# ZGC-SP/mpcith_kyber_kosk

Measured on AMD Instinct MI355X. Metric: kyber768_kosk_proofs_per_sec_prove_plus_verify, higher is better.
Workload: dtype u16

## Files before the change

### include/kosk_mi355x.h

```cpp
#ifndef KOSK_MI355X_H
#define KOSK_MI355X_H

#include <stddef.h>
#include <stdint.h>

#ifdef __cplusplus
extern "C" {
#endif

typedef struct kosk_ctx kosk_ctx;

typedef void (*kosk_randombytes_fn)(void *user, uint8_t *out, size_t len);

size_t kosk_pk_bytes(int kyber_k);
size_t kosk_sk_bytes(int kyber_k);
size_t kosk_proof_bytes(int kyber_k);
size_t kosk_tape_bytes(int kyber_k);
int kosk_proof_field(int kyber_k, int idx, size_t *offset, size_t *size);

#define KOSK_SEED_BYTES 32
int kosk_tape_from_seed(int kyber_k, const uint8_t seed[KOSK_SEED_BYTES], uint8_t *tape);

int kosk_create(kosk_ctx **ctx, int device, int kyber_k, int max_batch);

// ... 51 lines not shown
                        const uint8_t *tapes, size_t tape_stride, uint8_t *pi);
int kosk_verify_inst(kosk_ctx *ctx, int n, const uint8_t *pi, const uint8_t *inst, uint8_t *ok);

int kosk_stage_prover_inputs(kosk_ctx *ctx, int n, const uint8_t *tapes, size_t tape_stride, uint8_t *pk, uint8_t *sk);
int kosk_prove_resident(kosk_ctx *ctx, int n);
int kosk_fetch_proofs(kosk_ctx *ctx, int n, uint8_t *pi);
int kosk_stage_verifier_inputs(kosk_ctx *ctx, int n, const uint8_t *pi, const uint8_t *pk);
int kosk_verify_resident(kosk_ctx *ctx, int n, uint8_t *ok);
int kosk_verifiable_keygen_resident(kosk_ctx *ctx, int n, const uint8_t *tapes, size_t tape_stride, uint8_t *pk, uint8_t *sk);
int kosk_verify_resident_pk(kosk_ctx *ctx, int n, const uint8_t *pk, uint8_t *ok);
size_t kosk_compact_proof_bytes(int kyber_k);
int kosk_proof_compress(int kyber_k, const uint8_t *pi, uint8_t *out);
int kosk_proof_decompress(int kyber_k, const uint8_t *in, uint8_t *pi);
int kosk_verifiable_keygen_batch_compact(kosk_ctx *ctx, int n, const uint8_t *tapes, size_t tape_stride,
                                         uint8_t *pk, uint8_t *sk, uint8_t *out);
int kosk_verify_batch_compact(kosk_ctx *ctx, int n, const uint8_t *in, const uint8_t *pk, uint8_t *ok);
int kosk_fetch_proofs_compact(kosk_ctx *ctx, int n, uint8_t *out);
int kosk_stage_verifier_inputs_compact(kosk_ctx *ctx, int n, const uint8_t *in, const uint8_t *pk);

size_t kosk_dense_proof_bytes(int kyber_k);
int kosk_proof_dense_pack(int kyber_k, const uint8_t *pi, uint8_t *out);
int kosk_proof_dense_unpack(int kyber_k, const uint8_t *in, uint8_t *pi);
int kosk_verifiable_keygen_batch_dense(kosk_ctx *ctx, int n, const uint8_t *tapes, size_t tape_stride, uint8_t *pk, uint8_t *sk, uint8_t *out);
int kosk_verifiable_keygen_seeded_batch_dense(kosk_ctx *ctx, int n, const uint8_t *seeds, size_t seed_stride, uint8_t *pk, uint8_t *sk,
                                              uint8_t *out);
int kosk_verify_batch_dense(kosk_ctx *ctx, int n, const uint8_t *in, const uint8_t *pk, uint8_t *ok);
int kosk_fetch_proofs_dense(kosk_ctx *ctx, int n, uint8_t *out);
int kosk_stage_verifier_inputs_dense(kosk_ctx *ctx, int n, const uint8_t *in, const uint8_t *pk);
int kosk_dense_fill_device(kosk_ctx *ctx, int n, uint8_t *d_images, size_t image_stride, uint32_t *d_status);

#define KOSK_SS_BYTES 32
size_t kosk_ct_bytes(int kyber_k);
int kosk_kem_enc_batch(kosk_ctx *ctx, int n, const uint8_t *pk, const uint8_t *coins, uint8_t *ct, uint8_t *ss);
int kosk_kem_dec_batch(kosk_ctx *ctx, int n, const uint8_t *ct, const uint8_t *sk, uint8_t *ss);
int kosk_kem_enc_verified(kosk_ctx *ctx, int n, const uint8_t *coins, uint8_t *ct, uint8_t *ss, uint8_t *done);

enum { KOSK_KEM_KEY_NONE = 0, KOSK_KEM_KEY_PK = 1, KOSK_KEM_KEY_SK = 2 };
int kosk_kem_key_set(kosk_ctx *ctx, const uint8_t *pk, const uint8_t *sk);
int kosk_kem_key_state(const kosk_ctx *ctx);
int kosk_kem_key_clear(kosk_ctx *ctx);
int kosk_kem_enc_key(kosk_ctx *ctx, int n, const uint8_t *coins, uint8_t *ct, uint8_t *ss);
int kosk_kem_dec_key(kosk_ctx *ctx, int n, const uint8_t *ct, uint8_t *ss);

int kosk_kem_keypair_batch(kosk_ctx *ctx, int n, const uint8_t *coins, uint8_t *pk, uint8_t *sk);
#define KOSK_KEYCHK_HASH     1
#define KOSK_KEYCHK_PK_RANGE 2
#define KOSK_KEYCHK_S_RANGE  4
int kosk_kem_check_pk(kosk_ctx *ctx, int n, const uint8_t *pk, uint8_t *flags);
int kosk_kem_check_sk(kosk_ctx *ctx, int n, const uint8_t *sk, uint8_t *flags);

int kosk_witness_from_sk(kosk_ctx *ctx, int n, const uint8_t *sk, int16_t *se_out, uint8_t *ok);
int kosk_stage_prover_keys(kosk_ctx *ctx, int n, const uint8_t *sk, const uint8_t *tapes, size_t tape_stride, uint8_t *ok);
int kosk_stage_prover_keys_seeded(kosk_ctx *ctx, int n, const uint8_t *sk, const uint8_t *seeds, size_t seed_stride, uint8_t *ok);
int kosk_prove_keys_batch(kosk_ctx *ctx, int n, const uint8_t *sk, const uint8_t *tapes, size_t tape_stride, uint8_t *pi, uint8_t *ok);
int kosk_prove_keys_seeded_batch(kosk_ctx *ctx, int n, const uint8_t *sk, const uint8_t *seeds, size_t seed_stride, uint8_t *pi, uint8_t *ok);

int kosk_path_count(const kosk_ctx *ctx, int id, long *count);
int kosk_host_threads(const kosk_ctx *ctx);

int kosk_phase_seconds(const kosk_ctx *ctx, double *out, int n);

int kosk_profile_enable(kosk_ctx *ctx, int on);
int kosk_profile_read(const kosk_ctx *ctx, int id, double *total_ms, long *launches);
int kosk_profile_read_units(const kosk_ctx *ctx, int id, double *total_ms, long *launches, long *proofs);

int kosk_combine_stats(const kosk_ctx *ctx, long *calls, long *members);

int kosk_stream_timer_start(kosk_ctx *ctx);
int kosk_stream_timer_stop(kosk_ctx *ctx, double *ms);


int kosk_sha3_256_batch(kosk_ctx *ctx, const uint8_t *d_in, size_t in_stride, size_t inlen, uint8_t *d_out, int n);
int kosk_sha3_256_batch_pair(kosk_ctx *ctx, const uint8_t *d_in, size_t in_stride, size_t inlen, uint8_t *d_out, int n);
int kosk_sha3_256_batch_wave(kosk_ctx *ctx, const uint8_t *d_in, size_t in_stride, size_t inlen, uint8_t *d_out, int n);
int kosk_fs_alpha_device(kosk_ctx *ctx, const uint8_t *d_tables, size_t table_stride, int n, uint16_t *d_alpha, uint8_t *d_h1);
int kosk_fs_opened_device(kosk_ctx *ctx, const uint8_t *d_tables, size_t table_stride, int n, uint16_t *d_sel, uint16_t *d_rest, int sel_stride, uint8_t *d_ch);
int kosk_shake256_batch(kosk_ctx *ctx, const uint8_t *d_in, size_t in_stride, size_t inlen,
                        uint8_t *d_out, size_t outlen, int n);
int kosk_tape_expand_device(kosk_ctx *ctx, int n, const uint8_t *seeds, size_t seed_stride, uint8_t *d_tapes, size_t tape_stride);
int kosk_commit_hash_lanes(kosk_ctx *ctx, const uint16_t *d_rows, size_t row_stride, int n_lanes,
                           const uint8_t *d_prefix, int with_prefix, uint8_t *d_out);
int kosk_ntt256_batch(kosk_ctx *ctx, const int16_t *d_in, int16_t *d_out, int n);
int kosk_lagrange_expand(kosk_ctx *ctx, const uint16_t *d_y407, uint16_t *d_shares, int n);
int kosk_recon_secrets(kosk_ctx *ctx, const uint16_t *d_shares, uint16_t *d_secrets, int n, int two_d);
int kosk_device_synchronize(kosk_ctx *ctx);
int kosk_streams(const kosk_ctx *ctx);
int kosk_resident_proofs(kosk_ctx *ctx, void **d_proofs, size_t *stride);
int kosk_resident_digests(kosk_ctx *ctx, int round, void **d_digests, size_t *stride);
typedef void (*kosk_round_fn)(void *user, int role, int round, const void *d_digests, size_t bytes);
int kosk_set_round_hook(kosk_ctx *ctx, kosk_round_fn fn, void *user);


int kosk_keygen(int kyber_k, const uint8_t seed64[64], uint8_t *pk, uint8_t *sk,
                int16_t *A, int16_t *s, int16_t *e, int16_t *t);
int kosk_fs_alpha(int kyber_k, const uint8_t *tcomm_all, uint16_t *alpha);
int kosk_fs_opened(const uint8_t *digests_all, uint16_t *I, uint16_t *rest);
void kosk_host_sha3_256(uint8_t out[32], const uint8_t *in, size_t inlen);
void kosk_host_shake256(uint8_t *out, size_t outlen, const uint8_t *in, size_t inlen);
int kosk_host_sha3_256_multi(uint8_t *out, const uint8_t *in, size_t in_stride, size_t inlen, int count, int nthreads);
int kosk_lagrange_table(int which, uint16_t *out);

int kosk_bind_value(int kyber_k, const uint8_t *pk, const uint8_t context[32], uint8_t out[32]);
int kosk_bind_device(kosk_ctx *ctx, int n, const uint8_t *pk, const uint8_t *contexts, size_t context_stride, uint8_t *d_out);
int kosk_fs_alpha_bound(int kyber_k, const uint8_t *tcomm_all, const uint8_t bind[32], uint16_t *alpha);
int kosk_fs_opened_bound(const uint8_t *digests_all, const uint8_t bind[32], uint16_t *I, uint16_t *rest);
int kosk_fs_alpha_bound_device(kosk_ctx *ctx, const uint8_t *d_tables, size_t table_stride, int n, const uint8_t *d_bind, uint16_t *d_alpha, uint8_t *d_h1);
int kosk_fs_opened_bound_device(kosk_ctx *ctx, const uint8_t *d_tables, size_t table_stride, int n, const uint8_t *d_bind,
                                uint16_t *d_sel, uint16_t *d_rest, int sel_stride, uint8_t *d_ch);
int kosk_set_contexts(kosk_ctx *ctx, int n, const uint8_t *contexts, size_t context_stride);

int kosk_keyseed_value(int kyber_k, const uint8_t *sk, const uint8_t *context, const uint8_t *salt, uint8_t seed[32]);
int kosk_keyseed_device(kosk_ctx *ctx, int n, const uint8_t *sk, const uint8_t *contexts, size_t context_stride,
                        const uint8_t *salts, size_t salt_stride, uint8_t *d_seeds);
int kosk_stage_prover_keys_derived(kosk_ctx *ctx, int n, const uint8_t *sk, const uint8_t *salts, size_t salt_stride, uint8_t *ok);
int kosk_prove_keys_derived_batch(kosk_ctx *ctx, int n, const uint8_t *sk, const uint8_t *salts, size_t salt_stride, uint8_t *pi, uint8_t *ok);

#ifdef __cplusplus
}
#endif
#endif
```

### mpcith_kyber_kosk_amd/api.py

```python
import ctypes as C
import os

from . import build as _build

_HERE = os.path.dirname(os.path.abspath(__file__))
LIB_PATH = os.environ.get("KOSK_LIB_PATH") or os.path.join(_HERE, "libkosk_mi355x.so")


class KoskError(RuntimeError):
    pass


def _load():
    if not os.path.exists(LIB_PATH):
        _build.build()
    lib = C.CDLL(LIB_PATH)
    u8p, u16p, i16p, sz, vp = C.POINTER(C.c_uint8), C.POINTER(C.c_uint16), C.POINTER(C.c_int16), C.c_size_t, C.c_void_p
    sig = {
        "kosk_pk_bytes": (sz, [C.c_int]), "kosk_sk_bytes": (sz, [C.c_int]),
        "kosk_proof_bytes": (sz, [C.c_int]), "kosk_tape_bytes": (sz, [C.c_int]),
        "kosk_proof_field": (C.c_int, [C.c_int, C.c_int, C.POINTER(sz), C.POINTER(sz)]),
        "kosk_create": (C.c_int, [C.POINTER(vp), C.c_int, C.c_int, C.c_int]),
        "kosk_options_init": (None, [vp]),
        "kosk_create_ex": (C.c_int, [C.POINTER(vp), C.c_int, C.c_int, C.c_int, vp]),
# ... 63 lines not shown
        "kosk_set_entropy": (C.c_int, [vp, C.c_int]),
        "kosk_tape_expand_device": (C.c_int, [vp, C.c_int, vp, sz, vp, sz]),
        "kosk_verifiable_keygen_seeded_batch": (C.c_int, [vp, C.c_int, vp, sz, vp, vp, vp]),
        "kosk_verifiable_keygen_seeded_batch_compact": (C.c_int, [vp, C.c_int, vp, sz, vp, vp, vp]),
        "kosk_verifiable_keygen_seeded_resident": (C.c_int, [vp, C.c_int, vp, sz, vp, vp]),
        "kosk_stage_prover_inputs_seeded": (C.c_int, [vp, C.c_int, vp, sz, vp, vp]),
    }
    if not (os.environ.get("KOSK_LIB_PATH") and not hasattr(lib, "kosk_tape_from_seed")):
        sig.update(seeded)
    kem = {
        "kosk_ct_bytes": (sz, [C.c_int]),
        "kosk_kem_enc_batch": (C.c_int, [vp, C.c_int, vp, vp, vp, vp]),
        "kosk_kem_dec_batch": (C.c_int, [vp, C.c_int, vp, vp, vp]),
        "kosk_kem_enc_verified": (C.c_int, [vp, C.c_int, vp, vp, vp, vp]),
    }
    if not (os.environ.get("KOSK_LIB_PATH") and not hasattr(lib, "kosk_kem_enc_batch")):
        sig.update(kem)
    keyproof = {
        "kosk_witness_from_sk": (C.c_int, [vp, C.c_int, vp, vp, vp]),
        "kosk_stage_prover_keys": (C.c_int, [vp, C.c_int, vp, vp, sz, vp]),
        "kosk_stage_prover_keys_seeded": (C.c_int, [vp, C.c_int, vp, vp, sz, vp]),
        "kosk_prove_keys_batch": (C.c_int, [vp, C.c_int, vp, vp, sz, vp, vp]),
        "kosk_prove_keys_seeded_batch": (C.c_int, [vp, C.c_int, vp, vp, sz, vp, vp]),
    }
    if not (os.environ.get("KOSK_LIB_PATH") and not hasattr(lib, "kosk_witness_from_sk")):
        sig.update(keyproof)
    bound = {
        "kosk_bind_value": (C.c_int, [C.c_int, vp, vp, vp]),
        "kosk_bind_device": (C.c_int, [vp, C.c_int, vp, vp, sz, vp]),
        "kosk_fs_alpha_bound": (C.c_int, [C.c_int, vp, vp, vp]),
        "kosk_fs_opened_bound": (C.c_int, [vp, vp, vp, vp]),
        "kosk_fs_alpha_bound_device": (C.c_int, [vp, vp, sz, C.c_int, vp, vp, vp]),
        "kosk_fs_opened_bound_device": (C.c_int, [vp, vp, sz, C.c_int, vp, vp, vp, C.c_int, vp]),
        "kosk_set_contexts": (C.c_int, [vp, C.c_int, vp, sz]),
    }
    if not (os.environ.get("KOSK_LIB_PATH") and not hasattr(lib, "kosk_set_contexts")):
        sig.update(bound)
    dense = {
        "kosk_dense_proof_bytes": (sz, [C.c_int]),
        "kosk_proof_dense_pack": (C.c_int, [C.c_int, vp, vp]),
        "kosk_proof_dense_unpack": (C.c_int, [C.c_int, vp, vp]),
        "kosk_fetch_proofs_dense": (C.c_int, [vp, C.c_int, vp]),
        "kosk_stage_verifier_inputs_dense": (C.c_int, [vp, C.c_int, vp, vp]),
        "kosk_verifiable_keygen_batch_dense": (C.c_int, [vp, C.c_int, vp, sz, vp, vp, vp]),
        "kosk_verifiable_keygen_seeded_batch_dense": (C.c_int, [vp, C.c_int, vp, sz, vp, vp, vp]),
        "kosk_verify_batch_dense": (C.c_int, [vp, C.c_int, vp, vp, vp]),
        "kosk_dense_fill_device": (C.c_int, [vp, C.c_int, vp, sz, vp]),
    }
    if not (os.environ.get("KOSK_LIB_PATH") and not hasattr(lib, "kosk_dense_proof_bytes")):
        sig.update(dense)
    keypair = {
        "kosk_kem_keypair_batch": (C.c_int, [vp, C.c_int, vp, vp, vp]),
        "kosk_kem_check_pk": (C.c_int, [vp, C.c_int, vp, vp]),
        "kosk_kem_check_sk": (C.c_int, [vp, C.c_int, vp, vp]),
    }
    if not (os.environ.get("KOSK_LIB_PATH") and not hasattr(lib, "kosk_kem_keypair_batch")):
        sig.update(keypair)
    keyseed = {
        "kosk_keyseed_value": (C.c_int, [C.c_int, vp, vp, vp, vp]),
        "kosk_keyseed_device": (C.c_int, [vp, C.c_int, vp, vp, sz, vp, sz, vp]),
        "kosk_stage_prover_keys_derived": (C.c_int, [vp, C.c_int, vp, vp, sz, vp]),
        "kosk_prove_keys_derived_batch": (C.c_int, [vp, C.c_int, vp, vp, sz, vp, vp]),
    }
    if not (os.environ.get("KOSK_LIB_PATH") and not hasattr(lib, "kosk_keyseed_value")):
        sig.update(keyseed)
    wipe = {
        "kosk_wipe_secrets": (C.c_int, [vp]),
        "kosk_set_wipe": (C.c_int, [vp, C.c_int]),
        "kosk_secret_scan": (C.c_int, [vp, vp, sz, C.POINTER(C.c_long)]),
        "kosk_wipe_device": (C.c_int, [vp, C.c_int, vp, vp]),
        "kosk_wipe_timing": (C.c_int, [vp, C.c_int, C.POINTER(C.c_double), C.POINTER(C.c_double), C.POINTER(C.c_size_t), C.POINTER(C.c_int)]),
    }
    if not (os.environ.get("KOSK_LIB_PATH") and not hasattr(lib, "kosk_wipe_secrets")):
        sig.update(wipe)
    onekey = {
        "kosk_kem_key_set": (C.c_int, [vp, vp, vp]),
        "kosk_kem_key_state": (C.c_int, [vp]),
        "kosk_kem_key_clear": (C.c_int, [vp]),
        "kosk_kem_enc_key": (C.c_int, [vp, C.c_int, vp, vp, vp]),
        "kosk_kem_dec_key": (C.c_int, [vp, C.c_int, vp, vp]),
    }
    if not (os.environ.get("KOSK_LIB_PATH") and not hasattr(lib, "kosk_kem_key_set")):
        sig.update(onekey)
    for name, (res, args) in sig.items():
        fn = getattr(lib, name)
        fn.restype = res
        fn.argtypes = args
    return lib


lib = _load()
EXPORTS = ["kosk_pk_bytes", "kosk_sk_bytes", "kosk_proof_bytes", "kosk_tape_bytes", "kosk_proof_field", "kosk_create",
           "kosk_destroy", "kosk_last_error", "kosk_set_randombytes", "kosk_verifiable_keygen_batch", "kosk_verify_batch",
           "kosk_verify_fail_masks", "kosk_randomness_bytes", "kosk_range_proof_bytes", "kosk_mlwe_inst_bytes",
           "kosk_prepare_randomness", "kosk_prepare_range_proof", "kosk_prove_prepared", "kosk_verify_inst", "kosk_compact_proof_bytes",
           "kosk_proof_compress", "kosk_proof_decompress", "kosk_fetch_proofs_compact", "kosk_stage_verifier_inputs_compact", "kosk_stage_prover_inputs", "kosk_prove_resident", "kosk_fetch_proofs",
           "kosk_stage_verifier_inputs", "kosk_verify_resident", "kosk_verifiable_keygen_resident", "kosk_verify_resident_pk",
           "kosk_resident_digests", "kosk_set_round_hook", "kosk_phase_seconds", "kosk_path_count", "kosk_host_threads", "kosk_sha3_256_batch_pair", "kosk_verifiable_keygen_batch_compact", "kosk_verify_batch_compact", "kosk_host_alloc", "kosk_host_free", "kosk_sha3_256_batch",
           "kosk_shake256_batch", "kosk_commit_hash_lanes", "kosk_ntt256_batch", "kosk_lagrange_expand",
           "kosk_recon_secrets", "kosk_profile_enable", "kosk_profile_read", "kosk_profile_read_units", "kosk_combine_stats", "kosk_stream_timer_start", "kosk_stream_timer_stop", "kosk_device_synchronize", "kosk_streams", "kosk_resident_proofs", "kosk_keygen", "kosk_fs_alpha",
           "kosk_fs_opened", "kosk_host_sha3_256", "kosk_host_shake256", "kosk_host_sha3_256_multi", "kosk_lagrange_table",
           "kosk_options_init", "kosk_create_ex", "kosk_sha3_256_batch_wave", "kosk_fs_alpha_device", "kosk_fs_opened_device",
           "kosk_tape_from_seed", "kosk_set_entropy", "kosk_tape_expand_device", "kosk_verifiable_keygen_seeded_batch",
           "kosk_verifiable_keygen_seeded_batch_compact", "kosk_verifiable_keygen_seeded_resident", "kosk_stage_prover_inputs_seeded",
           "kosk_ct_bytes", "kosk_kem_enc_batch", "kosk_kem_dec_batch", "kosk_kem_enc_verified",
           "kosk_witness_from_sk", "kosk_stage_prover_keys", "kosk_stage_prover_keys_seeded", "kosk_prove_keys_batch",
           "kosk_prove_keys_seeded_batch",
           "kosk_bind_value", "kosk_bind_device", "kosk_fs_alpha_bound", "kosk_fs_opened_bound", "kosk_fs_alpha_bound_device",
           "kosk_fs_opened_bound_device", "kosk_set_contexts",
           "kosk_dense_proof_bytes", "kosk_proof_dense_pack", "kosk_proof_dense_unpack", "kosk_fetch_proofs_dense",
           "kosk_stage_verifier_inputs_dense", "kosk_verifiable_keygen_batch_dense", "kosk_verifiable_keygen_seeded_batch_dense",
           "kosk_verify_batch_dense", "kosk_dense_fill_device",
           "kosk_kem_keypair_batch", "kosk_kem_check_pk", "kosk_kem_check_sk",
           "kosk_keyseed_value", "kosk_keyseed_device", "kosk_stage_prover_keys_derived", "kosk_prove_keys_derived_batch",
           "kosk_wipe_secrets", "kosk_set_wipe", "kosk_secret_scan", "kosk_wipe_device", "kosk_wipe_timing",
           "kosk_kem_key_set", "kosk_kem_key_state", "kosk_kem_key_clear", "kosk_kem_enc_key", "kosk_kem_dec_key"]
HAS_KEM = hasattr(lib, "kosk_kem_enc_batch")


class KoskOptions(C.Structure):
    _fields_ = [("size", C.c_uint32), ("streams", C.c_int32), ("combine", C.c_int32), ("combine_wait_us", C.c_int32),
                ("combine_idle_us", C.c_int32), ("combine_prewake_us", C.c_int32), ("strict_encoding", C.c_int32), ("fs_mode", C.c_int32),
                ("host_threads", C.c_int32), ("blocking_sync", C.c_int32), ("hooks_unmerged", C.c_int32), ("reserved", C.c_int32 * 6)]


FS_HOST, FS_DEVICE = 0, 1
ENTROPY_TAPE, ENTROPY_SEED = 0, 1
WIPE_OFF, WIPE_CALL = 0, 1
SEED_BYTES = 32
SS_BYTES = 32
KEYPAIR_COIN_BYTES = 64
KEYCHK_HASH, KEYCHK_PK_RANGE, KEYCHK_S_RANGE = 1, 2, 4
KEM_KEY_NONE, KEM_KEY_PK, KEM_KEY_SK = 0, 1, 2


def options(**fields):
    o = KoskOptions()
    lib.kosk_options_init(C.byref(o))
    for k_, v_ in fields.items():
        if k_ not in dict(KoskOptions._fields_) or k_ in ("size", "reserved"):
            raise KoskError("unknown option " + k_)
        setattr(o, k_, int(v_))
    return o


def pk_bytes(k): return lib.kosk_pk_bytes(k)
def sk_bytes(k): return lib.kosk_sk_bytes(k)
def proof_bytes(k): return lib.kosk_proof_bytes(k)
def tape_bytes(k): return lib.kosk_tape_bytes(k)
def ct_bytes(k): return lib.kosk_ct_bytes(k)
def dense_proof_bytes(k): return lib.kosk_dense_proof_bytes(k)


def dense_pack(k, pi):
    if len(pi) != proof_bytes(k):
        raise KoskError("dense_pack: an image of kosk_proof_bytes")
    out = C.create_string_buffer(dense_proof_bytes(k))
    rc = lib.kosk_proof_dense_pack(k, C.c_char_p(bytes(pi)), out)
    return rc, out.raw


def dense_unpack(k, rec):
    if len(rec) != dense_proof_bytes(k):
        raise KoskError("dense_unpack: a record of kosk_dense_proof_bytes")
    out = C.create_string_buffer(proof_bytes(k))
    rc = lib.kosk_proof_dense_unpack(k, C.c_char_p(bytes(rec)), out)
    return rc, out.raw


CONTEXT_BYTES = 32


def bind_value(k, pk, context):
    pk, context = bytes(pk), bytes(context)
    if len(pk) != pk_bytes(k) or len(context) != CONTEXT_BYTES:
        raise KoskError("bind_value: a public key of kosk_pk_bytes and a context of %d bytes" % CONTEXT_BYTES)
    out = C.create_string_buffer(32)
    if lib.kosk_bind_value(k, C.c_char_p(pk), C.c_char_p(context), out):
        raise KoskError("kosk_bind_value: kyber_k outside 2..4")
    return out.raw


SALT_BYTES = 32


def keyseed_value(k, sk, context=None, salt=None):
    sk = bytes(sk)
    if len(sk) != sk_bytes(k):
        raise KoskError("keyseed_value: a secret key of kosk_sk_bytes")
    if context is not None and len(context) != CONTEXT_BYTES:
        raise KoskError("a context has %d bytes" % CONTEXT_BYTES)
    if salt is not None and len(salt) != SALT_BYTES:
        raise KoskError("a salt has %d bytes" % SALT_BYTES)
    out = C.create_string_buffer(SEED_BYTES)
    cp = None if context is None else C.c_char_p(bytes(context))
    sp = None if salt is None else C.c_char_p(bytes(salt))
    if lib.kosk_keyseed_value(k, C.c_char_p(sk), cp, sp, out):
        raise KoskError("kosk_keyseed_value: kyber_k outside 2..4")
    return out.raw
# ... 331 lines not shown
    def verify_inst(self, proofs, insts):
        n = len(proofs)
        ok = (C.c_uint8 * n)()
        self._chk(lib.kosk_verify_inst(self._h, n, b"".join(proofs), b"".join(insts), ok), "verify_inst")
        return [bool(x) for x in ok]

    def stage_prover_inputs(self, tapes=None, n=None, seeds=None, seed_stride=None):
        if seeds is not None:
            sp, ss, n, _keep = self._seed_arg(seeds, n, seed_stride)
            self._pk = C.create_string_buffer(self.pk_bytes * n); self._sk = C.create_string_buffer(self.sk_bytes * n)
            self._chk(lib.kosk_stage_prover_inputs_seeded(self._h, n, sp, ss, self._pk, self._sk), "stage_prover_inputs")
            return n
        if tapes is not None:
            n = len(tapes)
        blob = b"".join(t[:self.tape_bytes] for t in tapes) if tapes is not None else None
        self._pk = C.create_string_buffer(self.pk_bytes * n); self._sk = C.create_string_buffer(self.sk_bytes * n)
        self._chk(lib.kosk_stage_prover_inputs(self._h, n, C.c_char_p(blob) if blob is not None else None, self.tape_bytes, self._pk, self._sk), "stage_prover_inputs")
        return n

    def prove_resident(self, n):
        self._chk(lib.kosk_prove_resident(self._h, n), "prove_resident")

    def verify_resident(self, n):
        ok = C.create_string_buffer(n)
        self._chk(lib.kosk_verify_resident(self._h, n, ok), "verify_resident")
        return [b == 1 for b in ok.raw]

    def fetch_proofs(self, n):
        pi = C.create_string_buffer(self.proof_bytes * n)
        self._chk(lib.kosk_fetch_proofs(self._h, n, pi), "fetch_proofs")
        return [pi.raw[i * self.proof_bytes:(i + 1) * self.proof_bytes] for i in range(n)]

    def verifiable_keygen_resident(self, tapes=None, n=None, tape_stride=None, seeds=None, seed_stride=None):
        if seeds is not None:
            sp, ss, n, _keep = self._seed_arg(seeds, n, seed_stride)
            if getattr(self, "_pk", None) is None or len(self._pk) != self.pk_bytes * n:
                self._pk = C.create_string_buffer(self.pk_bytes * n); self._sk = C.create_string_buffer(self.sk_bytes * n)
            self._chk(lib.kosk_verifiable_keygen_seeded_resident(self._h, n, sp, ss, self._pk, self._sk), "verifiable_keygen_resident")
            return n
        if isinstance(tapes, int):
            tp, stride = C.c_void_p(tapes), tape_stride
        elif tapes is None:
            tp, stride = None, 0
        else:
            n = len(tapes)
            blob = b"".join(t[:self.tape_bytes] for t in tapes)
            tp, stride = C.c_char_p(blob), self.tape_bytes
        if getattr(self, "_pk", None) is None or len(self._pk) != self.pk_bytes * n:
            self._pk = C.create_string_buffer(self.pk_bytes * n); self._sk = C.create_string_buffer(self.sk_bytes * n)
        self._chk(lib.kosk_verifiable_keygen_resident(self._h, n, tp, stride, self._pk, self._sk), "verifiable_keygen_resident")
        return n

    def keys(self, n):
        return ([self._pk.raw[i * self.pk_bytes:(i + 1) * self.pk_bytes] for i in range(n)],
                [self._sk.raw[i * self.sk_bytes:(i + 1) * self.sk_bytes] for i in range(n)])

    def verify_resident_pk(self, n, pks=None):
        ok = C.create_string_buffer(n)
        self._chk(lib.kosk_verify_resident_pk(self._h, n, C.c_char_p(b"".join(pks)) if pks is not None else None, ok), "verify_resident_pk")
        return [b == 1 for b in ok.raw]

    def resident_digests(self, rnd, n):
        d, stride = C.c_void_p(), C.c_size_t()
        self._chk(lib.kosk_resident_digests(self._h, rnd, C.byref(d), C.byref(stride)), "resident_digests")
        assert stride.value == 1454 * 32
        return DeviceView(d.value, (n, 1454, 32))

    def set_round_hook(self, fn):
        if fn is None:
            self._hook = None
            self._chk(lib.kosk_set_round_hook(self._h, None, None), "set_round_hook")
            return
        CB = C.CFUNCTYPE(None, C.c_void_p, C.c_int, C.c_int, C.c_void_p, C.c_size_t)
        self._hook = CB(lambda _u, role, rnd, ptr, nbytes: fn(role, rnd, ptr, nbytes))
        self._chk(lib.kosk_set_round_hook(self._h, C.cast(self._hook, C.c_void_p), None), "set_round_hook")

    def phase_seconds(self):
        out = (C.c_double * 16)()
        lib.kosk_phase_seconds(self._h, out, 16)
        return list(out)

    PROFILE_IDS = ["hash_tcomm", "hash_view", "gemm_expand1", "gemm_expand2", "lincomb", "ntt_f", "assemble",
                   "v_hash_tcomm", "v_hash_view", "v_interp_build", "v_gemm_interp", "v_gemm_expand", "v_gemm_recon", "v_lincomb",
                   "fs_alpha", "fs_opened", "v_fs_alpha", "v_fs_opened"]

    def profile_enable(self, on=True):
        self._chk(lib.kosk_profile_enable(self._h, int(on)), "profile_enable")

    def profile_read(self):
        out = {}
        for i, name in enumerate(self.PROFILE_IDS):
            ms, cnt = C.c_double(), C.c_long()
            lib.kosk_profile_read(self._h, i, C.byref(ms), C.byref(cnt))
            out[name] = (ms.value, cnt.value)
        return out

    def profile_read_units(self):
        out = {}
        for i, name in enumerate(self.PROFILE_IDS):
            ms, cnt, units = C.c_double(), C.c_long(), C.c_long()
            lib.kosk_profile_read_units(self._h, i, C.byref(ms), C.byref(cnt), C.byref(units))
            out[name] = (ms.value, cnt.value, units.value)
        return out

    def combine_stats(self):
        a, b = C.c_long(), C.c_long()
        self._chk(lib.kosk_combine_stats(self._h, C.byref(a), C.byref(b)), "combine_stats")
        return a.value, b.value

    def _records(self, what, x, n, size):
        if isinstance(x, int):
            if n is None:
                raise KoskError("a device pointer for %s needs n" % what)
            return C.c_void_p(x), n, None
        for r_ in x:
            if len(r_) != size:
                raise KoskError("a %s record has %d bytes" % (what, size))
        blob = b"".join(bytes(r_) for r_ in x)
        return C.c_char_p(blob), len(x), blob

    def _kem_out(self, out, n, sizes):
        if out is not None:
            if len(out) != len(sizes):
                raise KoskError("out needs %d device pointers" % len(sizes))
            return [C.c_void_p(int(p_)) for p_ in out], None
        bufs = [C.create_string_buffer(s_ * n) for s_ in sizes]
        return bufs, bufs

    def kem_enc(self, pks, coins=None, n=None, out=None):
        pp, n, _k1 = self._records("pk", pks, n, self.pk_bytes)
        cp, _k2 = None, None
        if coins is not None:
            cp, nc, _k2 = self._records("coins", coins, n, 32)
            if nc != n:
                raise KoskError("coins for %d items, public keys for %d" % (nc, n))
        ctb = ct_bytes(self.k)
        bufs, host = self._kem_out(out, n, (ctb, SS_BYTES))
        self._chk(lib.kosk_kem_enc_batch(self._h, n, pp, cp, bufs[0], bufs[1]), "kem_enc")
        if host is None:
            return out
        return _cut(bufs[0], ctb, n), _cut(bufs[1], SS_BYTES, n)

    def kem_dec(self, cts, sks, n=None, out=None):
        ctb = ct_bytes(self.k)
        cp, n, _k1 = self._records("ct", cts, n, ctb)
        sp, ns, _k2 = self._records("sk", sks, n, self.sk_bytes)
        if ns != n:
            raise KoskError("secret keys for %d items, ciphertexts for %d" % (ns, n))
        bufs, host = self._kem_out(None if out is None else (out,), n, (SS_BYTES,))
        self._chk(lib.kosk_kem_dec_batch(self._h, n, cp, sp, bufs[0]), "kem_dec")
        if host is None:
            return out
        return _cut(bufs[0], SS_BYTES, n)

    def kem_keypair(self, coins=None, n=None, out=None):
        cp, _k = None, None
        if coins is not None:
            cp, n, _k = self._records("coins", coins, n, KEYPAIR_COIN_BYTES)
        elif n is None:
            n = 1
        bufs, host = self._kem_out(out, n, (self.pk_bytes, self.sk_bytes))
        self._chk(lib.kosk_kem_keypair_batch(self._h, n, cp, bufs[0], bufs[1]), "kem_keypair")
        if host is None:
            return out
        return _cut(bufs[0], self.pk_bytes, n), _cut(bufs[1], self.sk_bytes, n)

    def _kem_check(self, fn, what, recs, n, size):
# ... 43 lines not shown
        self._chk(lib.kosk_kem_enc_key(self._h, n, cp, bufs[0], bufs[1]), "kem_enc_key")
        if host is None:
            return out
        return _cut(bufs[0], ctb, n), _cut(bufs[1], SS_BYTES, n)

    def kem_dec_key(self, cts, n=None, out=None):
        ctb = ct_bytes(self.k)
        cp, n, _k = self._records("ct", cts, n, ctb)
        bufs, host = self._kem_out(None if out is None else (out,), n, (SS_BYTES,))
        self._chk(lib.kosk_kem_dec_key(self._h, n, cp, bufs[0]), "kem_dec_key")
        if host is None:
            return out
        return _cut(bufs[0], SS_BYTES, n)

    def witness_from_sk(self, sks, n=None):
        import numpy as np
        sp, n, _keep = self._records("sk", sks, n, self.sk_bytes)
        se = np.zeros((n, 2 * self.k, 256), np.int16)
        ok = C.create_string_buffer(n)
        self._chk(lib.kosk_witness_from_sk(self._h, n, sp, se.ctypes.data, ok), "witness_from_sk")
        return se, [b == 1 for b in ok.raw[:n]]

    def _key_rand(self, tapes, seeds, n, seed_stride):
        if seeds is not None:
            sp, ss, ns, keep = self._seed_arg(seeds, n, seed_stride)
            if ns != n:
                raise KoskError("seeds for %d proofs, secret keys for %d" % (ns, n))
            return True, sp, ss, keep
        if tapes is None:
            return False, None, 0, None
        if isinstance(tapes, int):
            return False, C.c_void_p(tapes), self.tape_bytes, None
        if len(tapes) != n:
            raise KoskError("tapes for %d proofs, secret keys for %d" % (len(tapes), n))
        for t in tapes:
            if len(t) < self.tape_bytes:
                raise KoskError("tape shorter than kosk_tape_bytes")
        blob = b"".join(t[:self.tape_bytes] for t in tapes)
        return False, C.c_char_p(blob), self.tape_bytes, blob

    def stage_prover_keys(self, sks, tapes=None, seeds=None, n=None, seed_stride=None, derived=False, salts=None, salt_stride=None):
        sp, n, _k1 = self._records("sk", sks, n, self.sk_bytes)
        if derived or salts is not None:
            if tapes is not None or seeds is not None:
                raise KoskError("derived=True takes neither tapes nor seeds")
            rp, stride, _k2 = self._salt_arg(salts, n, salt_stride)
            ok = C.create_string_buffer(n)
            self._chk(lib.kosk_stage_prover_keys_derived(self._h, n, sp, rp, stride, ok), "stage_prover_keys")
            return [b == 1 for b in ok.raw[:n]]
        seeded, rp, stride, _k2 = self._key_rand(tapes, seeds, n, seed_stride)
        ok = C.create_string_buffer(n)
        fn = lib.kosk_stage_prover_keys_seeded if seeded else lib.kosk_stage_prover_keys
        self._chk(fn(self._h, n, sp, rp, stride, ok), "stage_prover_keys")
        return [b == 1 for b in ok.raw[:n]]

    def prove_keys(self, sks, tapes=None, seeds=None, n=None, seed_stride=None, derived=False, salts=None, salt_stride=None):
        sp, n, _k1 = self._records("sk", sks, n, self.sk_bytes)
        if derived or salts is not None:
            if tapes is not None or seeds is not None:
                raise KoskError("derived=True takes neither tapes nor seeds")
            rp, stride, _k2 = self._salt_arg(salts, n, salt_stride)
            ok = C.create_string_buffer(n)
            pi = C.create_string_buffer(self.proof_bytes * n)
            self._chk(lib.kosk_prove_keys_derived_batch(self._h, n, sp, rp, stride, pi, ok), "prove_keys")
            return _cut(pi, self.proof_bytes, n), [b == 1 for b in ok.raw[:n]]
        seeded, rp, stride, _k2 = self._key_rand(tapes, seeds, n, seed_stride)
        ok = C.create_string_buffer(n)
        pi = C.create_string_buffer(self.proof_bytes * n)
        fn = lib.kosk_prove_keys_seeded_batch if seeded else lib.kosk_prove_keys_batch
        self._chk(fn(self._h, n, sp, rp, stride, pi, ok), "prove_keys")
        return _cut(pi, self.proof_bytes, n), [b == 1 for b in ok.raw[:n]]

    PATH_IDS = ["hash_dma", "hash_plain", "table_gemm", "limb_gemm", "copy_direct", "copy_staged", "graph_replay", "digest_copy", "small_copy_kernel",
                "fs_device", "fs_host", "tape_expand", "kem_enc", "kem_dec"]

    PATH_DENSE_FILL = 14
    PATH_KEM_KEYPAIR = 15
    PATH_KEM_CHECK = 16
    PATH_KEYSEED = 17
    PATH_WIPE = 18
    PATH_KEM_KEY_SETUP = 19
    PATH_KEM_ENC_KEY = 20
    PATH_KEM_DEC_KEY = 21

    def path_count(self, path_id):
        v = C.c_long()
        self._chk(lib.kosk_path_count(self._h, int(path_id), C.byref(v)), "path_count")
        return v.value

    def path_counts(self):
        out = {}
        for i, name in enumerate(self.PATH_IDS if HAS_KEM else self.PATH_IDS[:12]):
            v = C.c_long()
            self._chk(lib.kosk_path_count(self._h, i, C.byref(v)), "path_count")
            out[name] = v.value
        return out

    @property
    def host_threads(self):
        return lib.kosk_host_threads(self._h)

    def timer_start(self):
        self._chk(lib.kosk_stream_timer_start(self._h), "timer_start")

    def timer_stop_ms(self):
        ms = C.c_double()
        self._chk(lib.kosk_stream_timer_stop(self._h, C.byref(ms)), "timer_stop")
        return ms.value

    @property
    def streams(self):
        return lib.kosk_streams(self._h)

    def synchronize(self):
        self._chk(lib.kosk_device_synchronize(self._h), "synchronize")

    def sha3_256_batch(self, d_in, in_stride, inlen, d_out, n):
        self._chk(lib.kosk_sha3_256_batch(self._h, d_in, in_stride, inlen, d_out, n), "sha3_256_batch")

    def sha3_256_batch_pair(self, d_in, in_stride, inlen, d_out, n):
        self._chk(lib.kosk_sha3_256_batch_pair(self._h, d_in, in_stride, inlen, d_out, n), "sha3_256_batch_pair")

    def sha3_256_batch_wave(self, d_in, in_stride, inlen, d_out, n):
        self._chk(lib.kosk_sha3_256_batch_wave(self._h, d_in, in_stride, inlen, d_out, n), "sha3_256_batch_wave")

    def fs_alpha_device(self, d_tables, table_stride, n, d_alpha, d_h1=None):
        self._chk(lib.kosk_fs_alpha_device(self._h, d_tables, table_stride, n, d_alpha, d_h1), "fs_alpha_device")

    def fs_opened_device(self, d_tables, table_stride, n, d_sel, d_rest, sel_stride, d_ch=None):
        self._chk(lib.kosk_fs_opened_device(self._h, d_tables, table_stride, n, d_sel, d_rest, sel_stride, d_ch), "fs_opened_device")

    def fs_alpha_bound_device(self, d_tables, table_stride, n, d_bind, d_alpha, d_h1=None):
        self._chk(lib.kosk_fs_alpha_bound_device(self._h, d_tables, table_stride, n, d_bind, d_alpha, d_h1), "fs_alpha_bound_device")

    def fs_opened_bound_device(self, d_tables, table_stride, n, d_bind, d_sel, d_rest, sel_stride, d_ch=None):
        self._chk(lib.kosk_fs_opened_bound_device(self._h, d_tables, table_stride, n, d_bind, d_sel, d_rest, sel_stride, d_ch), "fs_opened_bound_device")

    def shake256_batch(self, d_in, in_stride, inlen, d_out, outlen, n):
        self._chk(lib.kosk_shake256_batch(self._h, d_in, in_stride, inlen, d_out, outlen, n), "shake256_batch")

    def commit_hash_lanes(self, d_rows, row_stride, n_lanes, d_prefix, with_prefix, d_out):
        self._chk(lib.kosk_commit_hash_lanes(self._h, d_rows, row_stride, n_lanes, d_prefix, int(with_prefix), d_out), "commit_hash_lanes")

    def ntt256_batch(self, d_in, d_out, n):
        self._chk(lib.kosk_ntt256_batch(self._h, d_in, d_out, n), "ntt256_batch")

    def lagrange_expand(self, d_y407, d_shares, n):
        self._chk(lib.kosk_lagrange_expand(self._h, d_y407, d_shares, n), "lagrange_expand")

    def recon_secrets(self, d_shares, d_secrets, n, two_d=False):
        self._chk(lib.kosk_recon_secrets(self._h, d_shares, d_secrets, n, int(two_d)), "recon_secrets")
```

### mpcith_kyber_kosk_amd/csrc/kosk_capi.cpp

```cpp
#include "../../include/kosk_mi355x.h"

#include <unistd.h>

#include <algorithm>
#include <condition_variable>
#include <cstdio>
#include <cstring>
#include <exception>
#include <functional>
#include <memory>
#include <mutex>
#include <string>
#include <thread>
#include <vector>

#include "kosk_combine.hpp"
#include "kosk_ctx.hpp"
#include "kosk_lanes.hpp"

using namespace kosk;

struct kosk_ctx;
struct Cohort {
    int device = 0, k = 0, per = 0;
// ... 1723 lines not shown
    return 0;
    GUARD_END
}
int kosk_fs_opened_bound_device(kosk_ctx *ctx, const uint8_t *d_tables, size_t table_stride, int n, const uint8_t *d_bind, uint16_t *d_sel, uint16_t *d_rest,
                                int sel_stride, uint8_t *d_ch)
{
    if (!ctx || !d_tables || !d_sel || !d_rest || !d_bind || n < 1 || sel_stride < NREST || sel_stride < SEL_OPOS + NOPEN ||
        (reinterpret_cast<uintptr_t>(d_tables) & 7) || (table_stride & 7) || (reinterpret_cast<uintptr_t>(d_bind) & 7)) return bad_args(ctx, __func__);
    GUARD(ctx)
    Ctx &c = *ctx->c;
    ctx->clear_err();
    HIPCHK_C(hipSetDevice(c.device));
    FsArgs fa{};
    fa.in = d_tables; fa.in_stride = table_stride; fa.len = NPARTY * 32; fa.out_digest = d_ch;
    fa.I = d_sel; fa.rest = d_rest; fa.sel_stride = sel_stride; fa.bind = d_bind;
    HIPCHK_C(launch_fs_chain(fa, FS_OPENED, n, c.stream));
    return 0;
    GUARD_END
}

int kosk_commit_hash_lanes(kosk_ctx *ctx, const uint16_t *d_rows, size_t row_stride, int n_lanes,
                           const uint8_t *d_prefix, int with_prefix, uint8_t *d_out)
{
    if (!ctx) return -1;
    GUARD(ctx)
    Ctx &c = *ctx->c;
    ctx->clear_err();
    HIPCHK_C(hipSetDevice(c.device));
    HashArgs ha{};
    ha.rows = d_rows;
    ha.group_stride = 0;
    ha.row_stride = (int)row_stride;
    ha.col_off = 0;
    ha.lanes_per_group = n_lanes;
    ha.prefix = d_prefix;
    ha.out = d_out;
    ha.out_lanes_per_group = n_lanes;
    int variant = 0;
    HIPCHK_C(launch_commit_hash(ha, 1, c.P.K, with_prefix != 0, c.stream, &variant));
    c.path_n[(variant & 1) ? PATH_HASH_DMA : PATH_HASH_PLAIN]++;
    return 0;
    GUARD_END
}

int kosk_ntt256_batch(kosk_ctx *ctx, const int16_t *d_in, int16_t *d_out, int n)
{
    if (!ctx) return -1;
    GUARD(ctx)
    Ctx &c = *ctx->c;
    ctx->clear_err();
    HIPCHK_C(hipSetDevice(c.device));
    NttArgs na{};
    na.in = d_in;
    na.out = d_out;
    na.npg = n;
    na.npoly = n;
    na.out_canonical = 0;
    HIPCHK_C(launch_ntt(na, c.stream));
    return 0;
    GUARD_END
}

int kosk_lagrange_expand(kosk_ctx *ctx, const uint16_t *d_y407, uint16_t *d_shares, int n)
{
    if (!ctx) return -1;
    GUARD(ctx)
    Ctx &c = *ctx->c;
    ctx->clear_err();
    HIPCHK_C(hipSetDevice(c.device));
    const int cap = c.own_batch * c.rm.nrows;
    for (int done = 0; done < n;) {
        const int m = (n - done) < cap ? (n - done) : cap;
        HIPCHK_C(launch_rows_copy(d_y407 + (size_t)done * XLEN, XLEN, c.d_P, RS, XLEN, m, c.stream));
        const GemmSrc gs{c.d_P, 0, nullptr, RS, 0, 0};
        const GemmDst gd{c.d_P, 0, nullptr, RS, EXP_OFF};
        if (gemm_modq(c, c.t_expand, gs, gd, m, 1)) return -1;
        HIPCHK_C(launch_rows_copy(c.d_P + NSEC, RS, d_shares + (size_t)done * NPARTY, NPARTY, NPARTY, m, c.stream));
        done += m;
    }
    return 0;
    GUARD_END
}

int kosk_recon_secrets(kosk_ctx *ctx, const uint16_t *d_shares, uint16_t *d_secrets, int n, int two_d)
{
    if (!ctx) return -1;
    GUARD(ctx)
    Ctx &c = *ctx->c;
    ctx->clear_err();
    HIPCHK_C(hipSetDevice(c.device));
    const GemmTable &t = two_d ? c.t_recon_2d : c.t_recon_d;
    const int cap = c.own_batch * c.rm.nrows;
    for (int done = 0; done < n;) {
        const int m = (n - done) < cap ? (n - done) : cap;
        HIPCHK_C(launch_rows_copy(d_shares + (size_t)done * NPARTY, NPARTY, c.d_P + NSEC, RS, NPARTY, m, c.stream));
        const GemmSrc gs{c.d_P, 0, nullptr, RS, NSEC, 0};
        const GemmDst gd{c.d_P, 0, nullptr, RS, 0};
        if (gemm_modq(c, t, gs, gd, m, 1)) return -1;
        HIPCHK_C(launch_rows_copy(c.d_P, RS, d_secrets + (size_t)done * NSEC, NSEC, NSEC, m, c.stream));
        done += m;
    }
    return 0;
    GUARD_END
}


int kosk_keygen(int kyber_k, const uint8_t seed64[64], uint8_t *pk, uint8_t *sk, int16_t *A, int16_t *s, int16_t *e, int16_t *t)
{
    Params P;
    if (!make_params(kyber_k, P) || !seed64 || !pk || !sk) return -1;
    return guard(static_cast<const kosk_ctx *>(nullptr), __func__, [&]() -> int {
    std::unique_ptr<HostKey> key(new HostKey());
    struct Gone { HostKey *k; ~Gone() { host_wipe(k, sizeof(HostKey)); } } gone{key.get()};
    host_keygen(P, seed64, pk, sk, *key);
    const int K = P.K;
    if (A) memcpy(A, key->A, sizeof(int16_t) * K * K * 256);
    if (s) memcpy(s, key->se, sizeof(int16_t) * K * 256);
    if (e) memcpy(e, key->se + K * 256, sizeof(int16_t) * K * 256);
    if (t) memcpy(t, key->t, sizeof(int16_t) * K * 256);
    return 0;
    GUARD_END
}

int kosk_fs_alpha(int kyber_k, const uint8_t *tcomm_all, uint16_t *alpha)
{
    Params P;
    if (!make_params(kyber_k, P) || !tcomm_all || !alpha) return -1;
    return guard(static_cast<const kosk_ctx *>(nullptr), __func__, [&]() -> int {
    fs_alpha(P, tcomm_all, alpha);
    return 0;
    GUARD_END
}

int kosk_fs_opened(const uint8_t *digests_all, uint16_t *I, uint16_t *rest)
{
    if (!digests_all || !I || !rest) return -1;
    return guard(static_cast<const kosk_ctx *>(nullptr), __func__, [&]() -> int {
    fs_opened(digests_all, I, rest);
    return 0;
    GUARD_END
}

int kosk_bind_value(int kyber_k, const uint8_t *pk, const uint8_t context[32], uint8_t out[32])
{
    Params P;
    if (!make_params(kyber_k, P) || !pk || !context || !out) return -1;
    return guard(static_cast<const kosk_ctx *>(nullptr), __func__, [&]() -> int {
    bind_value(P, pk, context, out);
    return 0;
    GUARD_END
}
int kosk_keyseed_value(int kyber_k, const uint8_t *sk, const uint8_t *context, const uint8_t *salt, uint8_t seed[32])
{
    Params P;
    if (!make_params(kyber_k, P) || !sk || !seed) return -1;
    return guard(static_cast<const kosk_ctx *>(nullptr), __func__, [&]() -> int {
    keyseed_value(P, sk, context, salt, seed);
    return 0;
    GUARD_END
}
int kosk_fs_alpha_bound(int kyber_k, const uint8_t *tcomm_all, const uint8_t bind[32], uint16_t *alpha)
{
    Params P;
    if (!make_params(kyber_k, P) || !tcomm_all || !bind || !alpha) return -1;
    return guard(static_cast<const kosk_ctx *>(nullptr), __func__, [&]() -> int {
    fs_alpha(P, tcomm_all, alpha, bind);
// ... 51 lines not shown
```

### mpcith_kyber_kosk_amd/csrc/kosk_ctx.cpp

```cpp
#include "kosk_ctx.hpp"

#include <atomic>

#include <chrono>
#include <cstdio>
#include <cstring>
#include <ctime>
#include <thread>

#include "kosk_math.hpp"

namespace kosk {

#define HIPCHK(x) KOSK_HIPCHK(x)

static double now_sec()
{
    return std::chrono::duration<double>(std::chrono::steady_clock::now().time_since_epoch()).count();
}

template <typename T>
static hipError_t dalloc(T **p, size_t n)
{
    return hipMalloc(reinterpret_cast<void **>(p), n * sizeof(T));
}
template <typename T>
static hipError_t halloc(T **p, size_t n)
{
    return hipHostMalloc(reinterpret_cast<void **>(p), n * sizeof(T), hipHostMallocDefault);
}

void Ctx::prof_collect()
{
    if (!prof_on) return;
    for (int i = 0; i < PR_COUNT; i++)
        if (prof_used[i]) {
            float ms = 0;
            if (hipEventElapsedTime(&ms, prof_ev[i][0], prof_ev[i][1]) == hipSuccess) { prof_ms[i] += ms; prof_n[i]++; prof_units[i] += prof_cur_units[i]; }
            prof_used[i] = false;
        }
}

Ctx::~Ctx()
{
    for (auto &g : seg)
        if (g.exec) (void)hipGraphExecDestroy(g.exec);
    for (auto &pe : prof_ev)
        for (auto e : pe)
            if (e) (void)hipEventDestroy(e);
    if (ev_sync) (void)hipEventDestroy(ev_sync);
    kem_release(*this);
    kem_key_release(*this);
    witness_release(*this);
    if (is_view) {
        if (h_err) (void)hipHostFree(h_err);
        if (d_compact) (void)hipFree(d_compact);
        if (d_compact_bad) (void)hipFree(d_compact_bad);
        if (h_compact) (void)hipHostFree(h_compact);
        if (h_compact_bad) (void)hipHostFree(h_compact_bad);
        if (d_dense_ws) (void)hipFree(d_dense_ws);
        if (d_dense_status) (void)hipFree(d_dense_status);
        if (pool) pool_destroy(pool);
        if (ev) (void)hipEventDestroy(ev);
        if (ev_kg) (void)hipEventDestroy(ev_kg);
        for (auto e : timer_ev)
            if (e) (void)hipEventDestroy(e);
        return;
    }
    void *dev[] = {t_expand.dfrag, t_recon_d.dfrag, t_recon_2d.dfrag, d_fresh_rows, d_gemm1_rows, d_gemm2_rows, d_off, d_fields, d_asm_groups, d_asm_elems,
                   d_rowtab, d_P, d_tape, d_seedbuf, d_dig1, d_dig2, d_proof, d_A, d_se, d_kg, d_sehat, d_t, d_alpha, d_I, d_pwT, d_coef, d_lin_rows,
                   d_gather, d_gather2, d_O, d_w, d_ell, d_sec, d_sec_u1, d_sec_u2, d_fail, d_inv, d_invlimb, d_vfields,
                   d_vrowtab, d_rows_bg, d_rows_isrc, d_rows_idst, d_rows_u, d_fact, d_invfact, d_node_of, d_isort, d_hrange, d_odig, d_bind};
    for (void *p : dev)
        if (p) (void)hipFree(p);
    void *host[] = {h_err, h_tape, h_seedbuf, h_dig, h_dig2, h_proof, h_alpha, h_I, h_fail, h_Iimg, h_kg, h_odig, h_bind};
    for (void *p : host)
        if (p) (void)hipHostFree(p);
    if (d_compact) (void)hipFree(d_compact);
    if (d_compact_bad) (void)hipFree(d_compact_bad);
    if (h_compact) (void)hipHostFree(h_compact);
    if (h_compact_bad) (void)hipHostFree(h_compact_bad);
    if (d_dense_ws) (void)hipFree(d_dense_ws);
    if (d_dense_status) (void)hipFree(d_dense_status);
    if (pool) pool_destroy(pool);
    if (ev) (void)hipEventDestroy(ev);
    if (ev_kg) (void)hipEventDestroy(ev_kg);
    for (auto e : timer_ev)
        if (e) (void)hipEventDestroy(e);
    if (stream) (void)hipStreamDestroy(stream);
}

static void pack_frag_table(const std::vector<uint16_t> &A, int M, int Kdim, int Mpad, int KS, std::vector<uint8_t> &out)
{
    const int RT = Mpad / 16;
    out.assign((size_t)KS * RT * 2048, 0);
    for (int m = 0; m < M; m++)
        for (int k = 0; k < Kdim; k++) {
            int c0, c1;
            limb_split(gf_center(A[(size_t)m * Kdim + k]), c0, c1);
            out[frag_offset(m, k, 0, RT)] = (uint8_t)(int8_t)c0;
            out[frag_offset(m, k, 1, RT)] = (uint8_t)(int8_t)c1;
        }
}

static int upload_table(Ctx &c, GemmTable &t, const std::vector<uint16_t> &A, int M, int Kdim)
{
    t.M = M;
    t.Mpad = (M + 127) / 128 * 128;
    t.KS = (Kdim + 63) / 64;
    std::vector<uint8_t> pk;
    pack_frag_table(A, M, Kdim, t.Mpad, t.KS, pk);
    HIPCHK(dalloc(&t.dfrag, pk.size()));
    c.reg_buf("table", &t.dfrag, pk.size(), 0);
    HIPCHK(hipMemcpyAsync(t.dfrag, pk.data(), pk.size(), hipMemcpyHostToDevice, c.stream));
    HIPCHK(hipStreamSynchronize(c.stream));
    return 0;
}

static hipError_t commit_hash_batch(Ctx &c, const HashArgs &ha, int n, int K, bool view, hipStream_t st)
{
    c.prof_begin(view ? PR_HASH_VIEW : PR_HASH_TCOMM, n);
    int variant = 0;
    const hipError_t e = launch_commit_hash(ha, n, K, view, st, &variant);
    if (!c.capturing) c.path_n[(variant & 1) ? PATH_HASH_DMA : PATH_HASH_PLAIN]++;
    c.prof_end(view ? PR_HASH_VIEW : PR_HASH_TCOMM);
    return e;
}

int device_error_check(Ctx &c)
{
    if (!c.h_err) return 0;
    const uint32_t e = *reinterpret_cast<volatile uint32_t *>(c.h_err);
    if (!e) return 0;
    *reinterpret_cast<volatile uint32_t *>(c.h_err) = 0;
    c.err = (e & DEVERR_XOF_BLOCKS) ? "gen_matrix: SHAKE128 block limit reached before 256 coefficients were accepted (indcpa.c:124-145 would squeeze on; "
                                      "probability < 2^-300 with the default limit of 32 blocks): no result was produced"
                                    : "a kernel reported an internal error";
    return -1;
}

int bind_check(Ctx &c, int n)
{
    if (c.bind_n > 0 && (c.bind_first < 0 || c.bind_first + n > c.bind_n)) {
        c.err = "the handle is armed with fewer contexts than this call has proofs (kosk_set_contexts)";
        return -1;
    }
    return 0;
}

int issue_bind_values(Ctx &c, int n)
{
    if (c.bind_n <= 0) return 0;
    if (bind_check(c, n)) return -1;
    BindArgs ba{};
    ba.pk = c.d_pk; ba.pk_stride = c.pk_stride; ba.pk_bytes = (int)c.P.pk_bytes; ba.K = c.P.K;
    ba.contexts = c.bind_ctx + (size_t)c.bind_first * 32;
    ba.out = c.d_bind;
    HIPCHK(launch_bind_values(ba, n, c.stream));
    if (!c.fs_device) HIPCHK(copy_small(c, c.h_bind, 0, c.d_bind, 0, (size_t)n * 32, 1, hipMemcpyDeviceToHost, c.stream));
    return 0;
}

hipError_t copy_round_table(Ctx &c, uint8_t *h_dst, const uint8_t *d_src, int n)
{
    return hipMemcpyAsync(h_dst, d_src, (size_t)n * NPARTY * 32, hipMemcpyDeviceToHost, c.stream);
}

hipError_t copy_small(Ctx &c, void *dst, size_t dst_stride, const void *src, size_t src_stride, size_t row_bytes, size_t nrows, hipMemcpyKind kind, hipStream_t st)
{
    if (!row_bytes || !nrows) return hipSuccess;
    if (copy_small_ok(src, src_stride, dst, dst_stride, row_bytes)) {
        if (!c.capturing) c.path_n[PATH_SMALL_COPY_KERNEL]++;
        return launch_copy_small(src, src_stride, dst, dst_stride, row_bytes, nrows, st);
    }
    if (nrows == 1 || (src_stride == row_bytes && dst_stride == row_bytes)) return hipMemcpyAsync(dst, src, row_bytes * nrows, kind, st);
    return hipMemcpy2DAsync(dst, dst_stride, src, src_stride, row_bytes, nrows, kind, st);
}

hipError_t stream_sync(Ctx &c)
{
    if (!c.blocking_sync) return hipStreamSynchronize(c.stream);
    const hipError_t e = hipEventRecord(c.ev_sync, c.stream);
    return e != hipSuccess ? e : hipEventSynchronize(c.ev_sync);
}

hipError_t wait_event(Ctx &c, hipEvent_t ev, int site, int n)
{
// ... 6 lines not shown
    if (!h) {
        h = lru;
        *h = Ctx::WaitHist{};
        h->n = n;
    }
    h->stamp = ++c.wait_stamp;
    int filled = 0;
    double est = 0;
    for (int i = 0; i < Ctx::WAIT_HIST; i++)
        if (h->us[i] > 0) { est = filled ? (h->us[i] < est ? h->us[i] : est) : h->us[i]; filled++; }
    const double t0 = now_sec();
    bool overslept = false;
    if (filled >= 4 && est > 250.0) {
        const double keep = est * 0.3 > 100.0 ? est * 0.3 : 100.0;
        double nap_us = est - keep;
        if (nap_us > 200000.0) nap_us = 200000.0;
        struct timespec ts;
        ts.tv_sec = 0;
        ts.tv_nsec = (long)(nap_us * 1e3);
        nanosleep(&ts, nullptr);
        const hipError_t q = hipEventQuery(ev);
        if (q == hipSuccess) overslept = true;
        else if (q != hipErrorNotReady) return q;
    }
    const hipError_t e = overslept ? hipSuccess : hipEventSynchronize(ev);
    const double took = (now_sec() - t0) * 1e6;
    if (overslept) {
        for (int i = 0; i < Ctx::WAIT_HIST; i++) h->us[i] = 0;
        h->at = 0;
    } else {
        h->us[h->at] = took > 1.0 ? took : 1.0;
        h->at = (h->at + 1) % Ctx::WAIT_HIST;
    }
    return e;
}
hipError_t stream_sync_site(Ctx &c, int site, int n)
{
    if (c.blocking_sync || !c.wait_nap) return stream_sync(c);
    const hipError_t e = hipEventRecord(c.ev_sync, c.stream);
    return e != hipSuccess ? e : wait_event(c, c.ev_sync, site, n);
}

int gemm_modq(Ctx &c, const GemmTable &t, const GemmSrc &s, const GemmDst &d, int npg, int ngroups)
{
    if (npg <= 0 || ngroups <= 0) return 0;
    GemmArgs ga{};
    ga.Afrag = t.dfrag; ga.Mpad = t.Mpad; ga.M = t.M; ga.KS = t.KS;
    ga.src = s.src; ga.src_gstride = s.gstride; ga.src_rows = s.rows; ga.src_rstride = s.rstride; ga.src_koff = s.koff;
    ga.src_canonical = s.canonical;
    ga.C = d.C; ga.c_gstride = d.gstride; ga.c_rows = d.rows; ga.c_rstride = d.rstride; ga.c_off = d.off;
    ga.npg = npg; ga.ngroups = ngroups;
    if (!table_gemm_ok(ga)) { c.err = "internal: table_gemm_ok() refuses the operands of a mod-q product"; return -1; }
    HIPCHK(launch_table_gemm(ga, c.stream));
    if (!c.capturing) c.path_n[PATH_TABLE_GEMM]++;
    return 0;
}

template <typename T>
static int upload_vec(Ctx &c, T **d, const std::vector<T> &v)
{
    HIPCHK(dalloc(d, v.size() ? v.size() : 1));
    c.reg_buf("table", d, v.size() * sizeof(T), 0);
    if (!v.empty()) {
        HIPCHK(hipMemcpyAsync(*d, v.data(), v.size() * sizeof(T), hipMemcpyHostToDevice, c.stream));
        HIPCHK(hipStreamSynchronize(c.stream));
    }
    return 0;
}

static int build_tables(Ctx &c)
{
    const Params &P = c.P;
    const RowMap &rm = c.rm;
    const int K = P.K, M = P.M, E = P.E, Z = P.Z;

    {
        std::vector<uint16_t> A((size_t)EXP_M * XLEN, 0);
        for (int m = 0; m < EXP_M; m++) {
            const int x = EXP_OFF + m;
            if (x < XLEN) A[(size_t)m * XLEN + x] = 1;
            else if (x < NPTS) lagrange_row(&A[(size_t)m * XLEN], XLEN, 0, x);
        }
        if (upload_table(c, c.t_expand, A, EXP_M, XLEN)) return -1;
    }
    {
        std::vector<uint16_t> A((size_t)NSEC * XLEN), A2((size_t)NSEC * (DEG2 + 1));
        for (int i = 0; i < NSEC; i++) {
            lagrange_row(&A[(size_t)i * XLEN], XLEN, NSEC, i);
            lagrange_row(&A2[(size_t)i * (DEG2 + 1)], DEG2 + 1, NSEC, i);
        }
        if (upload_table(c, c.t_recon_d, A, NSEC, XLEN)) return -1;
        if (upload_table(c, c.t_recon_2d, A2, NSEC, DEG2 + 1)) return -1;
    }

    std::vector<int16_t> fresh;
    for (int i = 0; i < M; i++) { fresh.push_back((int16_t)(rm.f + i)); fresh.push_back((int16_t)(rm.tf + i)); }
    for (int i = 0; i < K; i++)
        for (int j = 0; j < E; j++) { fresh.push_back((int16_t)(rm.seta + i * E + j)); fresh.push_back((int16_t)(rm.eeta + i * E + j)); }
    for (int i = 0; i < K; i++) { fresh.push_back((int16_t)(rm.s + i)); fresh.push_back((int16_t)(rm.e + i)); }
    for (int i = 0; i < K; i++) fresh.push_back((int16_t)(rm.nttas + i));
    for (int i = 0; i < K; i++)
        for (int j = 0; j < Z; j++) { fresh.push_back((int16_t)rm.zs(i, j)); fresh.push_back((int16_t)rm.ze(i, j)); }
    if ((int)fresh.size() != P.nfresh) { c.err = "internal: fresh row count"; return -1; }
    if (upload_vec(c, &c.d_fresh_rows, fresh)) return -1;
    if (upload_vec(c, &c.d_gemm1_rows, fresh)) return -1;
    c.n_gemm1 = (int)fresh.size();
    std::vector<int16_t> g2;
    for (int i = 0; i < K; i++) { g2.push_back((int16_t)(rm.nttsr + i)); g2.push_back((int16_t)(rm.ntter + i)); g2.push_back((int16_t)(rm.nttasr + i)); }
    if (upload_vec(c, &c.d_gemm2_rows, g2)) return -1;
    c.n_gemm2 = (int)g2.size();

    {
        std::vector<int16_t> lr(256, 0);
        for (int j = 0; j < P.J; j++) {
            lr[j] = (int16_t)(j < NCHK ? rm.beta(j) : rm.r + (j - NCHK));
            lr[128 + j] = (int16_t)(j < NCHK ? rm.gamma(j) : rm.nttr + (j - NCHK));
        }
        if (upload_vec(c, &c.d_lin_rows, lr)) return -1;
    }

    std::vector<int32_t> off;
    auto push_rows = [&](int row0, int n) { int b = (int)off.size(); for (int i = 0; i < n; i++) off.push_back((row0 + i) * RS); return b; };
    c.off_ntt1_src = push_rows(rm.f, M);
    push_rows(rm.s, K);
    c.off_ntt1_dst = push_rows(rm.tf, M);
    push_rows(rm.shat, K);
    c.n_ntt1 = M + K;
    c.off_sr_er = push_rows(rm.sr, 2 * K);
    c.off_nttsr_er = push_rows(rm.nttsr, 2 * K);
    if (rm.er != rm.sr + K || rm.ntter != rm.nttsr + K) { c.err = "internal: row map adjacency"; return -1; }
    if (upload_vec(c, &c.d_off, off)) return -1;

    auto add = [&](int fid, int sel, int width, auto rowfn) {
        FieldDesc fd{};
        fd.off = (uint32_t)P.off[fid];
        fd.sel = sel;
        fd.width = width;
        fd.rowtab_off = (int)c.h_rowtab.size();
        for (int e = 0; e < width; e++) c.h_rowtab.push_back((int16_t)rowfn(e));
        c.h_fields.push_back(fd);
    };
    add(F_F, 0, M, [&](int e) { return rm.f + e; });
    add(F_NTTF, 0, M, [&](int e) { return rm.tf + e; });
    add(F_BETA, 1, NCHK, [&](int e) { return rm.beta(e); });
    add(F_GAMMA, 1, NCHK, [&](int e) { return rm.gamma(e); });
    add(F_S, 0, K, [&](int e) { return rm.s + e; });
    add(F_E, 0, K, [&](int e) { return rm.e + e; });
    add(F_T, 1, K, [&](int e) { return rm.t + e; });
    add(F_NTTS, 0, K, [&](int e) { return rm.ntts + e; });
    add(F_NTTE, 0, K, [&](int e) { return rm.ntte + e; });
    add(F_NTTAR, 0, K, [&](int e) { return rm.nttar + e; });
    add(F_NTTAS, 0, K, [&](int e) { return rm.nttas + e; });
    add(F_SR, 1, K, [&](int e) { return rm.sr + e; });
    add(F_ER, 1, K, [&](int e) { return rm.er + e; });
    add(F_SETA, 1, K * E, [&](int e) { return rm.seta + e; });
    add(F_EETA, 1, K * E, [&](int e) { return rm.eeta + e; });
    add(F_SSUB, 0, K * E, [&](int e) { return rm.ssub + e; });
    add(F_ESUB, 0, K * E, [&](int e) { return rm.esub + e; });
    add(F_ZS, 0, K * Z, [&](int e) { return rm.zs(e / Z, e % Z); });
    add(F_ZE, 0, K * Z, [&](int e) { return rm.ze(e / Z, e % Z); });
    add(F_US, 1, K * Z, [&](int e) { return rm.us(e / Z, e % Z); });
    add(F_UE, 1, K * Z, [&](int e) { return rm.ue(e / Z, e % Z); });
    c.nfields = (int)c.h_fields.size();
    c.pplan = make_field_plan(c.h_fields.data(), c.nfields);
    {
        std::vector<AsmGroup> groups;
        std::vector<AsmElem> elems;
        for (int sel = 1; sel >= 0; sel--) {
            AsmGroup g{};
            auto flush = [&]() {
                if (g.nsub) groups.push_back(g);
                g = AsmGroup{};
            };
            for (int f = 0; f < c.nfields; f++) {
                const FieldDesc &fd = c.h_fields[f];
                if (fd.sel != sel) continue;
                if (g.nsub && (g.nrows + fd.width > 80 || g.nsub == 12)) flush();
                if (!g.nsub) { g.sel = sel; g.rowtab_off = (int)c.h_rowtab.size(); g.elem_off = (int)elems.size(); }
                g.sub_off[g.nsub] = fd.off; g.sub_width[g.nsub] = (int16_t)fd.width; g.sub_col[g.nsub] = (int16_t)g.nrows;
                for (int k = 0; k < fd.width; k++) {
                    c.h_rowtab.push_back(c.h_rowtab[fd.rowtab_off + k]);
                    elems.push_back(AsmElem{(int32_t)(fd.off / 2 + k), (int16_t)fd.width, (int16_t)(64 * g.nrows + k)});
                }
                g.nrows += fd.width;
                g.nsub++;
            }
            flush();
        }
        if ((int)groups.size() > ASM_MAX_GROUPS) { c.err = "internal: image field groups"; return -1; }
        for (int i = 0; i < 128; i++) elems.push_back(AsmElem{0, 1, 0});
        c.n_asm_groups = (int)groups.size();
        if (upload_vec(c, &c.d_asm_groups, groups)) return -1;
        if (upload_vec(c, &c.d_asm_elems, elems)) return -1;
    }
    if (upload_vec(c, &c.d_fields, c.h_fields)) return -1;
    if (upload_vec(c, &c.d_rowtab, c.h_rowtab)) return -1;
    return 0;
}

int ctx_create(Ctx **out, int device, int kyber_k, int max_batch, std::string &err, int host_share, const CtxOpts &opts)
{
    Ctx *cp = new Ctx();
    Ctx &c = *cp;
    auto fail = [&]() { err = c.err; delete cp; return -1; };
    if (!make_params(kyber_k, c.P)) { c.err = "kyber_k must be 2, 3 or 4"; return fail(); }
    if (max_batch < 1) { c.err = "max_batch must be >= 1"; return fail(); }
    int ndev = 0;
    if (hipGetDeviceCount(&ndev) != hipSuccess || ndev <= 0) {
        (void)hipGetLastError();
        c.err = "no HIP device available: the KOSK path has no CPU fallback";
        return fail();
    }
    if (device < 0 || device >= ndev) {
        c.err = "device " + std::to_string(device) + " out of range: " + std::to_string(ndev) + " HIP device(s) visible";
        return fail();
    }
    c.device = device;
    c.max_batch = max_batch;
    c.rm = make_rowmap(c.P);
    const int cpus = host_cpu_count() / (host_share > 0 ? host_share : 1);
    c.nthreads = cpus > 8 ? 8 : (cpus < 1 ? 1 : cpus);
    if (opts.host_threads > 0) c.nthreads = opts.host_threads > 64 ? 64 : opts.host_threads;
    c.pool = pool_create();
    c.nthreads = pool_reserve(c.pool, c.nthreads);
    c.base_threads = c.nthreads;
    c.reserved_threads = c.nthreads;
    c.own_batch = max_batch;
    c.call_cap = max_batch;
    if (const char *e = getenv("KOSK_GRAPHS")) c.use_graphs = atoi(e) != 0;
    if (const char *e = getenv("KOSK_WAIT_NAP")) c.wait_nap = atoi(e) != 0;
    if (const char *e = getenv("KOSK_REGISTER")) c.host_register = atoi(e) != 0;
    if (const char *e = getenv("KOSK_DEBUG_XOF_BLOCKS")) c.xof_max_blocks = atoi(e) > 0 ? atoi(e) : c.xof_max_blocks;
    if (opts.blocking_sync >= 0) c.blocking_sync = opts.blocking_sync != 0;
    if (opts.strict_encoding >= 0) c.strict_encoding = opts.strict_encoding != 0;
    if (opts.fs_device >= 0) c.fs_device = opts.fs_device != 0;

    auto body = [&]() -> int {
        HIPCHK(hipSetDevice(device));
        {
            int cus = 0;
            HIPCHK(hipDeviceGetAttribute(&cus, hipDeviceAttributeMultiprocessorCount, device));
            if (cus > 0) c.n_simd = 4 * cus;
        }
        HIPCHK(hipStreamCreateWithFlags(&c.stream, hipStreamNonBlocking));
        HIPCHK(hipEventCreateWithFlags(&c.ev, hipEventDisableTiming | (c.blocking_sync ? hipEventBlockingSync : 0)));
        HIPCHK(hipEventCreateWithFlags(&c.ev_kg, hipEventDisableTiming | (c.blocking_sync ? hipEventBlockingSync : 0)));
        if (c.blocking_sync) HIPCHK(hipEventCreateWithFlags(&c.ev_sync, hipEventDisableTiming | hipEventBlockingSync));
        else if (c.wait_nap) HIPCHK(hipEventCreateWithFlags(&c.ev_sync, hipEventDisableTiming));
        for (auto &pe : c.prof_ev)
            for (auto &e : pe) HIPCHK(hipEventCreate(&e));
        if (build_tables(c)) return -1;
        const Params &P = c.P;
        const size_t B = (size_t)max_batch;
        c.proof_stride = (size_t)c.rm.nrows * RS;
        c.tape_stride = (P.tape_bytes + 63) / 64 * 64;
        c.image_stride = (P.proof_bytes + 63) / 64 * 64;
        c.key_stride = (size_t)P.K * P.K * 256;
        c.se_stride = (size_t)2 * P.K * 256;
        c.sel_stride = 1312;
        auto dev = [&](auto **p, size_t per) -> hipError_t {
            const hipError_t e = dalloc(p, B * per);
            if (e == hipSuccess) { c.reg_pp(p, per * sizeof(**p)); c.reg_buf("workspace", p, per * sizeof(**p), Ctx::INV_PER_PROOF); }
            return e;
        };
        auto host = [&](auto **p, size_t per) -> hipError_t {
// ... 800 lines not shown
```

### mpcith_kyber_kosk_amd/csrc/kosk_ctx.hpp

```cpp
#pragma once
#include <hip/hip_runtime.h>

#include <string>
#include <functional>
#include <vector>

#include "kosk_device.hpp"
#include "kosk_host.hpp"
#include "kosk_params.hpp"

#define KOSK_HIPCHK(x)                                                      \
    do {                                                                    \
        hipError_t e_ = (x);                                                \
        if (e_ != hipSuccess) {                                             \
            (void)hipGetLastError();                                        \
            c.err = std::string(#x) + ": " + hipGetErrorString(e_);         \
            return -1;                                                      \
        }                                                                   \
    } while (0)

namespace kosk {

typedef void (*randombytes_fn)(void *user, uint8_t *out, size_t len);
typedef void (*round_fn)(void *user, int role, int round, const void *d_digests, size_t bytes);

struct KeygenIn {
    const uint8_t *tapes;
    size_t tape_stride;
    uint8_t *pk, *sk;
    int count = 0;
    const KeygenIn *next = nullptr;
    round_fn hook = nullptr;
    void *hook_user = nullptr;
    const uint8_t *seeds = nullptr;
    size_t seed_stride = 0;
};
struct VerifySeg {
    int count;
    const uint8_t *pk;
    uint8_t *ok;
    const VerifySeg *next = nullptr;
    round_fn hook = nullptr;
    void *hook_user = nullptr;
};

enum Phase { PH_HOST_PRE = 0, PH_GPU_COMMIT, PH_FS_ALPHA, PH_GPU_RELATION, PH_FS_OPEN, PH_GPU_ASSEMBLE, PH_D2H,
             PH_P1_ISSUE, PH_P2_ISSUE, PH_P3_ISSUE, PH_V1_ISSUE, PH_V1_WAIT, PH_V_FS_ALPHA, PH_V2_ISSUE, PH_V2_WAIT, PH_V_FS_OPEN,
             PH_COUNT };

enum ProfId { PR_HASH_TCOMM = 0, PR_HASH_VIEW, PR_GEMM_EXPAND1, PR_GEMM_EXPAND2, PR_LINCOMB, PR_NTT_F, PR_ASSEMBLE,
              PR_V_HASH_TCOMM, PR_V_HASH_VIEW, PR_V_INTERP_BUILD, PR_V_GEMM_INTERP, PR_V_GEMM_EXPAND, PR_V_GEMM_RECON,
              PR_V_LINCOMB, PR_FS_ALPHA, PR_FS_OPENED, PR_V_FS_ALPHA, PR_V_FS_OPENED, PR_COUNT };

enum PathId { PATH_HASH_DMA = 0, PATH_HASH_PLAIN, PATH_TABLE_GEMM, PATH_LIMB_GEMM, PATH_COPY_DIRECT, PATH_COPY_STAGED,
              PATH_GRAPH_REPLAY, PATH_DIGEST_COPY, PATH_SMALL_COPY_KERNEL, PATH_FS_DEVICE, PATH_FS_HOST, PATH_TAPE_EXPAND, PATH_KEM_ENC, PATH_KEM_DEC, PATH_DENSE_FILL, PATH_KEM_KEYPAIR, PATH_KEM_CHECK, PATH_KEYSEED, PATH_WIPE,
              PATH_KEM_KEY_SETUP, PATH_KEM_ENC_KEY, PATH_KEM_DEC_KEY, PATH_COUNT };

struct GemmTable {
    uint8_t *dfrag = nullptr;
    int M = 0, Mpad = 0, KS = 0;
};

struct GemmSrc {
    const uint16_t *src;
    size_t gstride;
    const int16_t *rows;
    int rstride, koff;
    int canonical = 1;
};
struct GemmDst {
    uint16_t *C;
    size_t gstride;
    const int16_t *rows;
    int rstride, off;
};

struct CompactField {
    uint32_t src_off, dst_off, n;
    int raw;
};
struct CompactPlan {
    CompactField f[NFIELDS];
    size_t bytes;
};
CompactPlan make_compact_plan(const Params &P);
int compact_encode(const Params &P, const uint8_t *img, uint8_t *out);
void compact_decode(const Params &P, const uint8_t *in, uint8_t *img);
CompactPlan make_dense_plan(const Params &P);
int dense_encode(const Params &P, const uint8_t *img, uint8_t *out);
int dense_decode(const Params &P, const uint8_t *in, uint8_t *img);

struct KemWs;
struct KemKey;
enum { KEM_CHUNK = 16384,
       KEM_WAVE_MAX = 1024 };

struct Ctx {
    int device = 0;
    Params P{};
    RowMap rm{};
    int max_batch = 0;
    struct PerProof { size_t field_off, stride_bytes; };
    std::vector<PerProof> per_proof;
    template <class T> void reg_pp(T **field, size_t stride_bytes)
    {
        per_proof.push_back({(size_t)(reinterpret_cast<char *>(field) - reinterpret_cast<char *>(this)), stride_bytes});
    }
    enum { INV_HOST = 1, INV_SECRET = 2, INV_PER_PROOF = 4 };
    enum { INVG_CORE = 0, INVG_VERIFY, INVG_COMPACT, INVG_DENSE, INVG_KEM, INVG_WITNESS, INVG_BIND, INVG_KEMKEY };
    struct InvBuf {
        const char *name;
        size_t field_off;
        void *abs;
        size_t bytes;
        size_t sec_off, sec_bytes;
        int flags, group;
    };
    std::vector<InvBuf> inv;
    template <class T> void reg_buf(const char *name, T **field, size_t bytes, int flags, int group = INVG_CORE, size_t sec_off = 0, size_t sec_bytes = (size_t)-1)
    {
        const char *f = reinterpret_cast<const char *>(field), *me = reinterpret_cast<const char *>(this);
        const bool mine = f >= me && f < me + sizeof(*this);
        inv.push_back(InvBuf{name, mine ? (size_t)(f - me) : (size_t)-1, mine ? nullptr : (void *)*field, bytes, sec_off, sec_bytes, flags, group});
    }
    template <class T> void inv_secret(const char *name, T **field, size_t sec_off = 0, size_t sec_bytes = (size_t)-1)
    {
        const size_t off = (size_t)(reinterpret_cast<const char *>(field) - reinterpret_cast<const char *>(this));
        for (InvBuf &b : inv)
            if (b.field_off == off) { b.name = name; b.flags |= INV_SECRET; b.sec_off = sec_off; b.sec_bytes = sec_bytes; }
    }
    void *inv_ptr(const InvBuf &b) const
    {
        return b.field_off == (size_t)-1 ? b.abs : *reinterpret_cast<void *const *>(reinterpret_cast<const char *>(this) + b.field_off);
    }
    void inv_drop(int group)
    {
        size_t k = 0;
        for (size_t i = 0; i < inv.size(); i++)
            if (inv[i].group != group) inv[k++] = inv[i];
        inv.resize(k);
    }
    bool staged_wiped = false;
    bool is_view = false;
    int view_first = 0;
    int own_batch = 0;
    int call_cap = 0;
    int base_threads = 1;
    int reserved_threads = 1;
    int nthreads = 1;
    Pool *pool = nullptr;
    hipStream_t stream = nullptr;
    std::string err;
    randombytes_fn rb = nullptr;
    void *rb_user = nullptr;
    bool entropy_seed = false;
    round_fn round_hook = nullptr;
    void *round_user = nullptr;

    GemmTable t_expand, t_recon_d, t_recon_2d;
    int16_t *d_fresh_rows = nullptr, *d_gemm1_rows = nullptr, *d_gemm2_rows = nullptr;
    int n_gemm1 = 0, n_gemm2 = 0;
    int32_t *d_off = nullptr;
    int off_ntt1_src = 0, off_ntt1_dst = 0, n_ntt1 = 0;
    int off_sr_er = 0, off_nttsr_er = 0;
    FieldDesc *d_fields = nullptr;
    int16_t *d_rowtab = nullptr;
    AsmGroup *d_asm_groups = nullptr;
    AsmElem *d_asm_elems = nullptr;
    int n_asm_groups = 0;
    int nfields = 0;
    std::vector<FieldDesc> h_fields;
    std::vector<int16_t> h_rowtab;

    size_t proof_stride = 0;
    size_t tape_stride = 0, image_stride = 0, key_stride = 0, se_stride = 0;
    int sel_stride = 0;
    uint16_t *d_P = nullptr;
    uint8_t *d_tape = nullptr, *d_dig1 = nullptr, *d_dig2 = nullptr, *d_proof = nullptr;
    const uint8_t *tape_cur = nullptr;
    size_t tape_cur_stride = 0;
    uint8_t *d_seedbuf = nullptr, *h_seedbuf = nullptr;
    TapeSegs tape_segs{};
    int16_t *d_A = nullptr, *d_se = nullptr;
    uint8_t *d_kg = nullptr, *h_kg = nullptr;
    size_t kg_rec = 0, sb_bytes = 0;
    uint8_t *d_seeds = nullptr, *d_pk = nullptr, *d_sb = nullptr;
    int16_t *d_sehat = nullptr;
    int resident_pk_n = 0;
    size_t pk_stride = 0, sb_stride = 0;
    unsigned long pk_epoch = 0;
    int keys_from_pk_n = 0;
    void note_pk_written(int n) { resident_pk_n = n; keys_from_pk_n = n; pk_epoch++; }
    void note_pk_decoded(int n) { if (n > keys_from_pk_n) keys_from_pk_n = n; }
    void note_keys_from_inst() { keys_from_pk_n = 0; pk_epoch++; }
    uint8_t *h_seeds = nullptr, *h_pk = nullptr, *h_sb = nullptr;
    uint16_t *d_t = nullptr;
    uint16_t *d_alpha = nullptr, *d_I = nullptr, *d_rest = nullptr;
    int32_t *d_pwT = nullptr;
    uint8_t *d_coef = nullptr;
    int16_t *d_lin_rows = nullptr;
    bool verify_ready = false;
    uint16_t *d_O = nullptr;
    size_t o_stride = 0;
    uint16_t *d_inv = nullptr;
    FieldDesc *d_vfields = nullptr;
    int16_t *d_vrowtab = nullptr;
    int n_vfields = 0;
    FieldPlan vplan{}, pplan{};
    int16_t *d_rows_bg = nullptr;
    int16_t *d_rows_isrc = nullptr, *d_rows_idst = nullptr;
    int16_t *d_rows_u = nullptr;
    int n_interp_d = 0, n_interp_2d = 0;
    uint16_t *d_w = nullptr, *d_ell = nullptr, *d_fact = nullptr, *d_invfact = nullptr;
    int16_t *d_node_of = nullptr;
    uint16_t *d_isort = nullptr, *d_hrange = nullptr;
    uint8_t *d_gather = nullptr, *d_gather2 = nullptr;
    uint16_t *d_invlimb = nullptr;
    uint16_t *d_sec = nullptr, *d_sec_u1 = nullptr, *d_sec_u2 = nullptr;
    uint32_t *d_fail = nullptr;
    uint16_t *h_Iimg = nullptr;
    uint8_t *d_odig = nullptr, *h_odig = nullptr;
    const uint8_t *host_img = nullptr;
    size_t host_img_stride = 0;
    hipEvent_t ev = nullptr;
    std::vector<uint16_t> v_I2, v_rest2;
    std::function<void()> near_end_hook;
    bool kg_on_host_pending = false;
    hipEvent_t ev_kg = nullptr;
    bool wait_nap = true;
    enum { WAIT_SITES = 8 };
    enum { WAIT_HIST = 8 };
    enum { WAIT_SIZES = 2 };
    struct WaitHist {
        int n = 0;
        int at = 0;
        unsigned long stamp = 0;
        double us[WAIT_HIST] = {0};
    };
    WaitHist wait_hist[WAIT_SITES][WAIT_SIZES];
    unsigned long wait_stamp = 0;
    hipEvent_t ev_sync = nullptr;
    bool blocking_sync = false;
    int n_simd = 1024;
    hipEvent_t timer_ev[2] = {nullptr, nullptr};
    CompactPlan cplan{};
    size_t compact_stride = 0;
    uint8_t *d_compact = nullptr, *h_compact = nullptr;
    uint32_t *d_compact_bad = nullptr, *h_compact_bad = nullptr;
    CompactPlan dplan{};
    size_t dense_stride = 0;
    uint16_t *d_dense_ws = nullptr;
    uint32_t *d_dense_status = nullptr;

    uint8_t *h_tape = nullptr, *h_dig = nullptr, *h_dig2 = nullptr, *h_proof = nullptr;
    uint16_t *h_alpha = nullptr, *h_I = nullptr, *h_rest = nullptr;
    uint32_t *h_fail = nullptr;
    uint32_t *h_err = nullptr;
    int xof_max_blocks = 32;
    XofGuard xof_guard() const { XofGuard g; g.err = h_err; g.max_blocks = xof_max_blocks; return g; }

    enum SegId { SEG_P1 = 0, SEG_P1B, SEG_P2, SEG_P2B, SEG_P3, SEG_V1, SEG_V1B, SEG_V2, SEG_V2B, SEG_COUNT };
    struct SegGraph {
        hipGraphExec_t exec = nullptr;
        int n = 0;
        const void *key_ptr = nullptr;
        size_t key_stride = 0;
    };
    SegGraph seg[SEG_COUNT];
    bool use_graphs = false;
    bool capturing = false;
    bool strict_encoding = true;
    bool fs_device = false;
    const uint8_t *bind_ctx = nullptr;
    int bind_n = 0, bind_first = 0;
    uint8_t *d_bind = nullptr, *h_bind = nullptr;
    bool host_register = true;
    long path_n[PATH_COUNT] = {0};
    KemWs *kem = nullptr;
    KemKey *kem_key = nullptr;

    double phase_sec[PH_COUNT] = {0};
    int prof_on = 0;
    hipEvent_t prof_ev[PR_COUNT][2] = {};
    bool prof_used[PR_COUNT] = {};
    double prof_ms[PR_COUNT] = {0};
    long prof_n[PR_COUNT] = {0};
    long prof_units[PR_COUNT] = {0};
    int prof_cur_units[PR_COUNT] = {0};
    void prof_begin(int id, int units = 0) { if (prof_on && !capturing) { (void)hipEventRecord(prof_ev[id][0], stream); prof_cur_units[id] = units; } }
    void prof_end(int id) { if (prof_on && !capturing) { (void)hipEventRecord(prof_ev[id][1], stream); prof_used[id] = true; } }
    void prof_collect();

    int wit_cap = 0;
    uint8_t *d_wsk = nullptr, *d_wok = nullptr, *h_wok = nullptr;
    uint8_t *d_wsalt = nullptr;
// ... 142 lines not shown
```

### mpcith_kyber_kosk_amd/csrc/kosk_device.hpp

```cpp
#pragma once
#include <hip/hip_runtime.h>

#include "kosk_math.hpp"
#include "kosk_params.hpp"

namespace kosk {

struct XofGuard {
    uint32_t *err = nullptr;
    int max_blocks = 32;
};
enum : uint32_t { DEVERR_XOF_BLOCKS = 1u };


struct HashArgs {
    const uint16_t *rows;
    size_t group_stride;
    int row_stride;
    int col_off;
    int lanes_per_group;
    const uint8_t *prefix;
    uint8_t *out;
    int out_lanes_per_group;
};

struct NttArgs {
    const int16_t *in;
    const int32_t *src_off;
    size_t in_gstride;
    int16_t *out;
    const int32_t *dst_off;
    size_t out_gstride;
    int npg;
    int npoly;
    int out_canonical;
    uint32_t *cmp_fail;
    int cmp_delta, cmp_bit;
    uint32_t npg_magic;
};
inline uint32_t ntt_npg_magic(int npg) { return npg <= 1 ? 0xFFFFFFFFu : (uint32_t)((1ull << 32) / (uint32_t)npg); }

KOSK_HD inline int limb_swz(int r) { return (-(r >> 2)) & 3; }
KOSK_HD inline size_t limb_offset(int r, int k, int limb, int RT)
{
    const int ks = k >> 6, kc = (k >> 4) & 3, rr = r & 15;
    return ((size_t)(ks * RT + (r >> 4)) * 2 + limb) * 1024 + rr * 64 + ((kc ^ limb_swz(rr)) << 4) + (k & 15);
}
KOSK_HD inline size_t frag_offset(int r, int k, int limb, int RT)
{
    return ((size_t)((k >> 6) * RT + (r >> 4)) * 2 + limb) * 1024 + (((k >> 4) & 3) * 16 + (r & 15)) * 16 + (k & 15);
}
KOSK_HD inline void limb_split(int32_t centred, int &c0, int &c1)
{
    c0 = ((centred + 32) & 63) - 32;
    c1 = (centred - c0) >> 6;
}
KOSK_HD inline uint16_t limb_pair(uint32_t v)
{
    int c0, c1;
    limb_split(gf_center(v), c0, c1);
    return (uint16_t)((c0 & 0xFF) | ((c1 & 0xFF) << 8));
}

struct GemmArgs {
    const uint8_t *Afrag;
    int Mpad, M, KS;
    const uint16_t *src;
    size_t src_gstride;
    const int16_t *src_rows;
    int src_rstride, src_koff;
    uint16_t *C;
    size_t c_gstride;
    const int16_t *c_rows;
    int c_rstride;
    int c_off;
    int npg;
    int src_canonical;
    int ngroups;
};

struct LincombArgs {
    uint16_t *P;
    size_t proof_stride;
    uint16_t *O;
    size_t o_stride;
    RowMap rm;
    int J;
    const int32_t *pwT;
    int ncols;
    const uint16_t *col_map;
    int col_map_stride;
    int nxb, njc, ngroups;
};

struct FieldDesc {
    uint32_t off;
    int sel;
    int width;
    int rowtab_off;
    int limit, limit_by_party;
    int noncanon_bit;
};

struct FieldPlan {
    uint8_t rest_ids[NFIELDS], open_ids[NFIELDS];
    int nrest, nopen;
};
inline FieldPlan make_field_plan(const FieldDesc *fields, int nfields)
{
    FieldPlan p{};
    for (int f = 0; f < nfields; f++) {
        if (fields[f].sel) p.rest_ids[p.nrest++] = (uint8_t)f;
        else p.open_ids[p.nopen++] = (uint8_t)f;
    }
    return p;
}

struct AsmElem {
    int32_t dst;
    int16_t width;
    int16_t tile;
};
struct AsmGroup {
    int sel;
    int nrows;
    int rowtab_off;
    int elem_off;
    int nsub;
    uint32_t sub_off[12];
    int16_t sub_width[12], sub_col[12];
};
constexpr int ASM_MAX_GROUPS = 8;

struct AssembleArgs {
    const uint16_t *P;
    size_t proof_stride;
    const int16_t *rowtab;
    const AsmGroup *groups;
    const AsmElem *elems;
    int ngroups;
    const uint16_t *opened, *rest;
    int sel_stride;
    const uint8_t *dig1, *dig2;
    uint8_t *proof;
    size_t image_stride;
    int img_align;
};

enum FailBit {
    FB_MALFORMED = 0, FB_BETA_GAMMA, FB_SR_ER_SHARES, FB_NTT_S_E, FB_A_SR, FB_T_PK, FB_T_RELATION,
    FB_ETA_CONST, FB_SUB_ETA, FB_U_INTERP, FB_U_RECON, FB_OPENED_SET
};

struct GateOffsets {
    uint32_t ssub, esub, zs, ze;
};

struct VerifyArgs {
    uint16_t *P;
    size_t proof_stride;
    uint16_t *O;
    size_t o_stride;
    RowMap rm;
// ... 70 lines not shown
    const uint8_t *sk;
    size_t sk_stride;
    const int16_t *A;
    size_t A_stride;
    const uint16_t *t;
    int16_t *se;
    size_t se_stride;
    uint8_t *pk;
    size_t pk_stride;
    uint8_t *ok;
};
bool witness_args_ok(const WitnessArgs &a);
hipError_t launch_witness_from_sk(const WitnessArgs &a, int n, hipStream_t st);

hipError_t launch_commit_hash(const HashArgs &a, int ngroups, int K, bool view, hipStream_t st, int *variant = nullptr);
hipError_t launch_sha3_msgs(const uint8_t *in, size_t in_stride, int len, uint8_t *out, size_t out_stride,
                            int outlen, int n, int domain, hipStream_t st);
hipError_t launch_sha3_msgs_pair(const uint8_t *in, size_t in_stride, int len, uint8_t *out, size_t out_stride, int outlen, int n,
                                 int domain, hipStream_t st);
enum FsMode { FS_DIGEST = 0, FS_ALPHA = 1, FS_OPENED = 2, FS_CHECK = 3 };
struct FsArgs {
    const uint8_t *in;
    size_t in_stride;
    int len;
    uint8_t *out_digest;
    uint16_t *alpha;
    int alpha_stride, J;
    uint16_t *I, *rest;
    int sel_stride;
    const uint8_t *proof;
    size_t image_stride;
    uint32_t off_I;
    uint32_t *fail;
    const uint8_t *bind;
};
struct BindArgs {
    const uint8_t *pk;
    size_t pk_stride;
    int pk_bytes, K;
    const uint8_t *contexts;
    uint8_t *out;
};
hipError_t launch_bind_values(const BindArgs &A, int n, hipStream_t st);
struct KeyseedArgs {
    const uint8_t *sk;
    size_t sk_stride;
    int sk_bytes, K;
    const uint8_t *contexts;
    size_t context_stride;
    const uint8_t *salts;
    size_t salt_stride;
    uint8_t *out;
};
hipError_t launch_keyseed(const KeyseedArgs &A, int n, hipStream_t st);
hipError_t launch_fs_chain(const FsArgs &A, int mode, int n, hipStream_t st);
bool copy_small_ok(const void *src, size_t src_stride, const void *dst, size_t dst_stride, size_t row_bytes);
hipError_t launch_copy_small(const void *src, size_t src_stride, void *dst, size_t dst_stride, size_t row_bytes, size_t nrows, hipStream_t st);
hipError_t launch_rows_copy(const uint16_t *src, size_t src_stride, uint16_t *dst, size_t dst_stride, int count,
                            int nrows, hipStream_t st);
struct TapeSegs {
    const uint8_t *ptr[16];
    int per, count;
};
struct KeygenFront {
    uint8_t *seeds;
    size_t seed_stride;
    int16_t *A;
    size_t A_stride;
    int16_t *se;
    size_t se_stride;
    XofGuard xof;
};
hipError_t launch_prover_pre(const uint8_t *tape, size_t tape_stride, uint16_t *P, size_t proof_stride, int row_f, int M,
                             int slice0_off, const int16_t *fresh_rows, int slice_begin, int slice_end, bool expand_f,
                             int witness_mode, const int16_t *se, size_t se_stride, const RowMap &rm, int eta1, int nproofs,
                             hipStream_t st, const KeygenFront *kg = nullptr, const TapeSegs *segs = nullptr);
hipError_t launch_ntt(const NttArgs &a, hipStream_t st);
hipError_t launch_relation_ntt(const NttArgs &na, const int16_t *A, size_t A_stride, uint16_t *P, size_t proof_stride, const RowMap &rm,
                               int nproofs, hipStream_t st);
hipError_t launch_matvec_ntt(const int16_t *A, size_t A_stride, uint16_t *P, size_t proof_stride, int v_row0, int row0, int K,
                             int nproofs, hipStream_t st);
bool table_gemm_ok(const GemmArgs &a);
hipError_t launch_table_gemm(const GemmArgs &a, hipStream_t st);
hipError_t launch_lincomb_stream(const uint16_t *P, size_t proof_stride, const RowMap &rm, const uint8_t *coef, uint16_t *C,
                                 const int16_t *lin_rows, int J, int nproofs, hipStream_t st);
hipError_t launch_coef_limbs(const uint16_t *alpha, int J, int M, uint8_t *B, int nproofs, hipStream_t st);
hipError_t launch_pow_table(const uint16_t *alpha, int J, int M, int32_t *pwT, int nproofs, hipStream_t st);
hipError_t launch_lincomb(const LincombArgs &a, int nproofs, hipStream_t st);
hipError_t launch_post_gates(uint16_t *P, size_t proof_stride, const RowMap &rm, int nproofs, hipStream_t st);
hipError_t launch_copy_tails(uint16_t *P, size_t proof_stride, const RowMap &rm, int nproofs, hipStream_t st);
hipError_t launch_post_relation(uint16_t *P, size_t proof_stride, const RowMap &rm, int nproofs, hipStream_t st);
hipError_t launch_assemble(const AssembleArgs &a, size_t off_tcomm, size_t off_comm, size_t off_I, int nproofs, hipStream_t st);

}
```

### mpcith_kyber_kosk_amd/csrc/kosk_kernels.hip

```cpp
#include <hip/hip_runtime.h>

#include <cstdlib>
#include <utility>

#include "kosk_device.hpp"
#include "kosk_keccak_dev.hpp"
#include "kosk_keccak_split_dev.hpp"
#include "kosk_keygen_dev.hpp"
#include "kosk_keygen_wave_dev.hpp"
#include "kosk_math.hpp"
#include "kosk_limb_dev.hpp"
#include "kosk_wave_sync_dev.hpp"

namespace kosk {

template <int PREFIX_WORDS, int NROWS, bool PIPE>
__global__ __launch_bounds__(64) void k_commit_hash(HashArgs a)
{
    const int lane = blockIdx.x * 64 + threadIdx.x;
    const int g = blockIdx.y;
    if (lane >= a.lanes_per_group) return;
    const uint16_t *__restrict__ base = a.rows + (size_t)g * a.group_stride + a.col_off + lane;
    const size_t dig = ((size_t)g * a.out_lanes_per_group + lane) * 32;

// ... 1156 lines not shown
    };
    for (int k0 = 0; k0 < M; k0 += 8) {
        uint32_t raw[8];
#pragma unroll
        for (int i = 0; i < 8; i++) raw[i] = in0[(size_t)(k0 + i < M ? k0 + i : M - 1) * istride];
#pragma unroll
        for (int i = 0; i < 4; i++) {
            const int k = k0 + 2 * i;
            if (k >= M) break;
            const uint32_t vv = centre_pair(raw[2 * i], raw[2 * i + 1]);
            const int32_t *pk = pw + (size_t)(k >> 1) * LC_JPAD;
#pragma unroll
            for (int j = 0; j < LC_JC; j++) asm("v_dot2_i32_i16 %0, %1, %2, %0" : "+v"(acc[j]) : "s"(pk[j]), "v"(vv));
        }
    }
    const uint32_t raw_chk = in0[0], raw_r = in0[(size_t)(NCHK + 1) * istride];
#pragma unroll
    for (int jj = 0; jj < LC_JC; jj++) {
        const int j = jc * LC_JC + jj;
        if (j >= a.J) break;
        int row;
        if (j < NCHK) row = which ? a.rm.gamma(j) : a.rm.beta(j);
        else row = (which ? a.rm.nttr : a.rm.r) + (j - NCHK);
        const uint32_t raw = j < NCHK ? raw_chk : raw_r;
        const uint32_t base = gf_fold(raw);
        uint32_t out = gf_from_i32(acc[jj] + (int32_t)base);
        if (raw >= (uint32_t)Q) {
            uint32_t sum = base;
            for (int k = 1; k < a.rm.M; k++) {
                const int32_t pp = pw[(size_t)(k >> 1) * LC_JPAD + jj];
                const int32_t pc = (k & 1) ? (pp >> 16) : (int32_t)(int16_t)(pp & 0xFFFF);
                sum += gf_mul((uint32_t)(pc < 0 ? pc + Q : pc), gf_fold(in0[(size_t)k * istride]));
            }
            const int nonwrap = (a.rm.M - 1) - (int)(sum / (uint32_t)Q), e0 = (int)(raw / (uint32_t)Q);
            if (e0 > nonwrap) out += (uint32_t)(e0 - nonwrap) * Q;
        }
        if (Ob) {
            Ob[(size_t)row * OS] = (uint16_t)out;
            if (j < NCHK && col < NSEC + XLEN) Pb[(size_t)row * RS + col] = (uint16_t)gf_fold(out);
        } else {
            Pb[(size_t)row * RS + col] = (uint16_t)out;
        }
    }
}


struct U16x8 {
    uint32_t v[8];
};
__device__ __forceinline__ U16x8 ld8(const uint16_t *p)
{
    const uint4 x = *reinterpret_cast<const uint4 *>(p);
    U16x8 r;
    r.v[0] = x.x & 0xFFFFu; r.v[1] = x.x >> 16; r.v[2] = x.y & 0xFFFFu; r.v[3] = x.y >> 16;
    r.v[4] = x.z & 0xFFFFu; r.v[5] = x.z >> 16; r.v[6] = x.w & 0xFFFFu; r.v[7] = x.w >> 16;
    return r;
}
__device__ __forceinline__ void st8(uint16_t *p, const U16x8 &r)
{
    *reinterpret_cast<uint4 *>(p) = make_uint4(r.v[0] | (r.v[1] << 16), r.v[2] | (r.v[3] << 16), r.v[4] | (r.v[5] << 16), r.v[6] | (r.v[7] << 16));
}

template <int E>
__global__ __launch_bounds__(256) void k_post_gates(uint16_t *__restrict__ P, size_t proof_stride, RowMap rm)
{
    const int x = threadIdx.x * 8, b = blockIdx.y;
    if (x >= NPTS) return;
    const int who = (int)blockIdx.z >= rm.K, i = blockIdx.z - (who ? rm.K : 0);
    uint16_t *Pb = P + (size_t)b * proof_stride + x;
    const U16x8 v = ld8(Pb + (size_t)((who ? rm.e : rm.s) + i) * RS);
    U16x8 c[E], zd[E - 1];
#pragma unroll
    for (int m = 0; m < E; m++) c[m] = ld8(Pb + (size_t)((who ? rm.eeta : rm.seta) + i * E + m) * RS);
#pragma unroll
    for (int m = 0; m < E - 1; m++) zd[m] = ld8(Pb + (size_t)(who ? rm.ze(i, m) : rm.zs(i, m)) * RS);
#pragma unroll
    for (int m = 0; m < E; m++) {
        U16x8 d, u;
#pragma unroll
        for (int q = 0; q < 8; q++) {
            d.v[q] = gf_sub(v.v[q], c[m].v[q]);
            if (m > 0) u.v[q] = gf_sub(gf_mul(m == 1 ? gf_sub(v.v[q], c[0].v[q]) : zd[m > 1 ? m - 2 : 0].v[q], d.v[q]), zd[m > 0 ? m - 1 : 0].v[q]);
        }
        st8(Pb + (size_t)((who ? rm.esub : rm.ssub) + i * E + m) * RS, d);
        if (m > 0) st8(Pb + (size_t)(who ? rm.ue(i, m - 1) : rm.us(i, m - 1)) * RS, u);
    }
}

__global__ __launch_bounds__(192) void k_copy_tails(uint16_t *__restrict__ P, size_t proof_stride, RowMap rm)
{
    const int t = threadIdx.x, i = blockIdx.x, b = blockIdx.y;
    if (t > NOPEN) return;
    uint16_t *Pb = P + (size_t)b * proof_stride + NSEC + t;
    const uint16_t s = Pb[(size_t)(rm.sr + i) * RS], e = Pb[(size_t)(rm.er + i) * RS];
    Pb[(size_t)(rm.nttsr + i) * RS] = s;
    Pb[(size_t)(rm.nttasr + i) * RS] = s;
    Pb[(size_t)(rm.ntter + i) * RS] = e;
}

__global__ __launch_bounds__(256) void k_post_relation(uint16_t *__restrict__ P, size_t proof_stride, RowMap rm)
{
    const int x = blockIdx.x * 256 + threadIdx.x, b = blockIdx.y;
    if (x >= NPTS) return;
    uint16_t *Pb = P + (size_t)b * proof_stride + x;
    for (int i = 0; i < rm.K; i++) {
        const uint32_t ns = gf_sub(Pb[(size_t)(rm.nttsr + i) * RS], Pb[(size_t)(rm.nttr + i) * RS]);
        const uint32_t ne = gf_sub(Pb[(size_t)(rm.ntter + i) * RS], Pb[(size_t)(rm.nttr + rm.K + i) * RS]);
        const uint32_t as = Pb[(size_t)(rm.nttas + i) * RS];
        Pb[(size_t)(rm.ntts + i) * RS] = (uint16_t)ns;
        Pb[(size_t)(rm.ntte + i) * RS] = (uint16_t)ne;
        Pb[(size_t)(rm.nttar + i) * RS] = (uint16_t)gf_sub(Pb[(size_t)(rm.nttasr + i) * RS], as);
        Pb[(size_t)(rm.t + i) * RS] = (uint16_t)gf_add(as, ne);
    }
}

constexpr int ASM_TILE = 64 * 80;

template <int MAXW>
__device__ __forceinline__ void asm_gather(const uint16_t *Pb, uint32_t voff, const int16_t *rt, int width, uint16_t *t, bool live)
{
    int rr[MAXW];
#pragma unroll
    for (int e = 0; e < MAXW; e++) rr[e] = rt[e < width ? e : width - 1];
    asm volatile("s_waitcnt vmcnt(0)" ::: "memory");
    __builtin_amdgcn_sched_barrier(0);
    uint32_t v[MAXW];
#pragma unroll
    for (int e = 0; e < MAXW; e++) {
        const int r = __builtin_amdgcn_readfirstlane(rr[e]);
        const uint16_t *rowp = Pb + (size_t)r * RS;
        asm volatile("global_load_ushort %0, %1, %2" : "=v"(v[e]) : "v"(voff), "s"(rowp));
    }
    asm volatile("s_waitcnt vmcnt(0)" ::: "memory");
    if (live) {
#pragma unroll
        for (int e = 0; e < MAXW; e++)
            if (e < width) t[e] = (uint16_t)v[e];
    }
}

template <int NQ>
__device__ __forceinline__ void asm_group_block(const AssembleArgs &a, const AsmGroup &g, const int b, const int w, uint16_t *tile, int16_t *rank_s,
                                                AsmElem *el_s)
{
    const int lane = threadIdx.x, slot = lane >> 4, cq = lane & 15;
    const uint16_t *orow = a.opened + (size_t)b * a.sel_stride;
    const uint16_t *Pb = a.P + (size_t)b * a.proof_stride;
    const int16_t *rt = a.rowtab + g.rowtab_off;
    uint16_t *img16 = reinterpret_cast<uint16_t *>(a.proof + (size_t)b * a.image_stride);
    const int nrows = g.nrows;
    const int lo = min(64 * w, NPARTY), hi = min(64 * (w + 1), NPARTY);
    const int i0 = orow[SEL_WIN + w], cnt = (int)orow[SEL_WIN + w + 1] - i0;
    const int k0 = lo - i0, nk = (hi - lo) - cnt;
    const int nsel = g.sel ? cnt : nk;
    if (nsel <= 0) return;
    rank_s[lane] = -1;
    int my_pos = 0;
    int my_col = 0;
    if (lane < nsel) {
        if (g.sel) my_col = (int)a.rest[(size_t)b * a.sel_stride + i0 + lane] - lo;
        else { my_col = (int)orow[SEL_OSORT + k0 + lane] - lo; my_pos = orow[SEL_OPOS + k0 + lane]; }
    }
    const AsmElem *el = a.elems + g.elem_off;
    el_s[lane] = el[lane];
    el_s[lane + 64] = el[lane + 64];
    __builtin_amdgcn_s_waitcnt(0);
    wave_lds_handoff();
    if (lane < nsel) rank_s[my_col] = (int16_t)lane;
    int rr[NQ];
#pragma unroll
    for (int q = 0; q < NQ; q++) rr[q] = rt[min(4 * q + slot, nrows - 1)];
    uint2 v[NQ];
    const uint16_t *src = Pb + NSEC + lo + 4 * cq;
#pragma unroll
    for (int q = 0; q < NQ; q++) v[q] = *reinterpret_cast<const uint2 *>(src + (size_t)rr[q] * RS);
    __builtin_amdgcn_s_waitcnt(0xC07F);
    wave_lds_handoff();
    int rk[4];
#pragma unroll
    for (int m = 0; m < 4; m++) rk[m] = rank_s[4 * cq + m];
#pragma unroll
    for (int q = 0; q < NQ; q++) {
        const int r = 4 * q + slot;
        if (r < nrows) {
            const uint32_t x[4] = {v[q].x & 0xFFFFu, v[q].x >> 16, v[q].y & 0xFFFFu, v[q].y >> 16};
            if (g.sel) {
                const AsmElem e = el_s[r];
#pragma unroll
                for (int m = 0; m < 4; m++)
                    if (rk[m] >= 0) tile[(int)e.tile + rk[m] * (int)e.width] = (uint16_t)x[m];
            } else {
#pragma unroll
                for (int m = 0; m < 4; m++)
                    if (rk[m] >= 0) tile[rk[m] * nrows + r] = (uint16_t)x[m];
            }
        }
    }
    __builtin_amdgcn_s_waitcnt(0);
    wave_lds_handoff();
    if (g.sel) {
        for (int s = 0; s < g.nsub; s++) {
            const int width = g.sub_width[s];
            uint16_t *out = img16 + g.sub_off[s] / 2 + (size_t)i0 * width;
            const uint16_t *srct = tile + 64 * (int)g.sub_col[s];
            const int n16 = cnt * width;
            const int head = (int)((reinterpret_cast<uintptr_t>(out) >> 1) & 1);
            const int body = (n16 - head) >> 1;
            if (lane == 0 && head) out[0] = srct[0];
            uint32_t *out32 = reinterpret_cast<uint32_t *>(out + head);
            for (int q = lane; q < body; q += 64) out32[q] = (uint32_t)srct[head + 2 * q] | ((uint32_t)srct[head + 2 * q + 1] << 16);
            if (lane == 1 && head + 2 * body < n16) out[n16 - 1] = srct[n16 - 1];
        }
    } else {
        const AsmElem e0 = el_s[lane], e1 = el_s[lane + 64];
        for (int j = 0; j < nk; j++) {
            const int i = __builtin_amdgcn_readlane(my_pos, j);
            if (lane < nrows) img16[e0.dst + i * (int)e0.width] = tile[j * nrows + lane];
            if (NQ > 16 && lane + 64 < nrows) img16[e1.dst + i * (int)e1.width] = tile[j * nrows + lane + 64];
        }
    }
}

__global__ __launch_bounds__(64) void k_assemble_groups(AssembleArgs a, uint32_t off_tcomm, uint32_t off_comm, uint32_t off_I, int blocks_per_proof, int nproofs)
{
    const int vid = xcd_virtual_id();
    const int b = vid / blocks_per_proof, bx = vid - b * blocks_per_proof;
    if (b >= nproofs) return;
    const int ngb = a.ngroups * NWIN;
    if (bx >= ngb) {
        const int q = (bx - ngb) * 64 + threadIdx.x;
        uint8_t *img = a.proof + (size_t)b * a.image_stride;
        if (q < NREST * 4) {
            const int i = q >> 2, tab = (q >> 1) & 1, half = q & 1;
            const size_t src = ((size_t)b * NPARTY + a.rest[(size_t)b * a.sel_stride + i]) * 32 + 16 * half;
            const uint4 v = *reinterpret_cast<const uint4 *>((tab ? a.dig2 : a.dig1) + src);
            uint8_t *dst = img + (tab ? off_comm : off_tcomm) + (size_t)i * 32 + 16 * half;
            if (a.img_align >= 16) *reinterpret_cast<uint4 *>(dst) = v;
            else if (a.img_align >= 8) {
                reinterpret_cast<uint2 *>(dst)[0] = make_uint2(v.x, v.y);
                reinterpret_cast<uint2 *>(dst)[1] = make_uint2(v.z, v.w);
            } else if (a.img_align >= 4) {
                const uint32_t w[4] = {v.x, v.y, v.z, v.w};
#pragma unroll
                for (int k = 0; k < 4; k++) reinterpret_cast<uint32_t *>(dst)[k] = w[k];
            } else {
                const uint32_t w[4] = {v.x, v.y, v.z, v.w};
#pragma unroll
                for (int k = 0; k < 8; k++) reinterpret_cast<uint16_t *>(dst)[k] = (uint16_t)(w[k >> 1] >> (16 * (k & 1)));
            }
        }
        if (q < NOPEN) reinterpret_cast<uint16_t *>(img + off_I)[q] = a.opened[(size_t)b * a.sel_stride + q];
        return;
    }
    __shared__ __attribute__((aligned(16))) uint16_t tile[ASM_TILE];
    __shared__ int16_t rank_s[64];
    __shared__ AsmElem el_s[128];
    const int gi = bx / NWIN, w = bx - gi * NWIN;
    const AsmGroup &g = a.groups[gi];
    if (g.nrows <= 16) asm_group_block<4>(a, g, b, w, tile, rank_s, el_s);
    else if (g.nrows <= 64) asm_group_block<16>(a, g, b, w, tile, rank_s, el_s);
    else asm_group_block<20>(a, g, b, w, tile, rank_s, el_s);
}

__global__ __launch_bounds__(256) void k_copy_small(const uint8_t *__restrict__ src, size_t src_stride, uint8_t *__restrict__ dst, size_t dst_stride,
                                                    uint32_t row_words, uint32_t nrows)
{
    const size_t total = (size_t)row_words * nrows;
    for (size_t i = (size_t)blockIdx.x * 256 + threadIdx.x; i < total; i += (size_t)gridDim.x * 256) {
        const uint32_t r = (uint32_t)(i / row_words), w = (uint32_t)(i - (size_t)r * row_words);
        reinterpret_cast<uint32_t *>(dst + (size_t)r * dst_stride)[w] = reinterpret_cast<const uint32_t *>(src + (size_t)r * src_stride)[w];
    }
}

__global__ __launch_bounds__(256) void k_rows_copy(const uint16_t *__restrict__ src, size_t src_stride,
                                                  uint16_t *__restrict__ dst, size_t dst_stride, int count)
{
    const int r = blockIdx.y;
    for (int x = blockIdx.x * 256 + threadIdx.x; x < count; x += gridDim.x * 256)
        dst[(size_t)r * dst_stride + x] = src[(size_t)r * src_stride + x];
}

template <int PW, int NR>
static int launch_hash_t(const HashArgs &a, int ngroups, hipStream_t st)
{
    dim3 grid((a.lanes_per_group + 63) / 64, ngroups);
    const long waves = (long)grid.x * grid.y;
    const bool dma_ok = a.row_stride % 8 == 0 && a.group_stride % 8 == 0 && a.col_off % 8 == 0 &&
                        (reinterpret_cast<uintptr_t>(a.rows) & 15) == 0 && a.col_off + (int)grid.x * 64 <= a.row_stride &&
                        (!PW || (reinterpret_cast<uintptr_t>(a.prefix) & 15) == 0);
    if (dma_ok) {
        const dim3 grid1((unsigned)waves);
        if (waves <= 2 * 1024 + 256) hipLaunchKernelGGL((k_commit_hash_dma<PW, NR, 2>), grid1, dim3(64), 0, st, a);
        else hipLaunchKernelGGL((k_commit_hash_dma<PW, NR, 1>), grid1, dim3(64), 0, st, a);
        return 1;
    }
    if (waves < 3 * 1024) hipLaunchKernelGGL((k_commit_hash<PW, NR, true>), grid, dim3(64), 0, st, a);
    else hipLaunchKernelGGL((k_commit_hash<PW, NR, false>), grid, dim3(64), 0, st, a);
    return 0;
}

hipError_t launch_commit_hash(const HashArgs &a, int ngroups, int K, bool view, hipStream_t st, int *variant)
// ... 242 lines not shown
```

### mpcith_kyber_kosk_amd/csrc/kosk_verify.cpp

```cpp
#include <atomic>
#include <cstring>
#include <functional>
#include <mutex>
#include <utility>
#include <vector>

#include "kosk_ctx.hpp"

#include <chrono>
#include "kosk_math.hpp"

namespace kosk {

static double now_sec()
{
    return std::chrono::duration<double>(std::chrono::steady_clock::now().time_since_epoch()).count();
}

#define HIPCHK(x) KOSK_HIPCHK(x)

template <typename T>
static hipError_t dalloc(T **p, size_t n) { return hipMalloc(reinterpret_cast<void **>(p), (n ? n : 1) * sizeof(T)); }
template <typename T>
static int upload_vec(Ctx &c, T **d, const std::vector<T> &v)
// ... 4 lines not shown
        HIPCHK(hipMemcpyAsync(*d, v.data(), v.size() * sizeof(T), hipMemcpyHostToDevice, c.stream));
        HIPCHK(hipStreamSynchronize(c.stream));
    }
    return 0;
}

int ensure_verify_workspace(Ctx &c)
{
    if (c.verify_ready) return 0;
    if (c.is_view) { c.err = "internal: a view's verifier workspace is allocated with its arena"; return -1; }
    const Params &P = c.P;
    const RowMap &rm = c.rm;
    const int K = P.K, M = P.M, E = P.E, Z = P.Z;
    const size_t B = (size_t)c.max_batch;

    std::vector<uint16_t> inv(Q + 1, 0);
    for (int a = 0; a < Q; a++) inv[a] = gf_inv_host((uint16_t)a);
    if (upload_vec(c, &c.d_inv, inv)) return -1;
    {
        const int len = interp_table_len(), off = interp_table_off();
        std::vector<uint16_t> il(len, 0);
        for (int i = 0; i + 2 < len; i++) il[i] = limb_pair(inv[((i - off) % Q + Q) % Q]);
        if (upload_vec(c, &c.d_invlimb, il)) return -1;
    }
    std::vector<uint16_t> fact(Q), invfact(Q);
    fact[0] = 1;
    for (int a = 1; a < Q; a++) fact[a] = (uint16_t)((uint32_t)fact[a - 1] * a % Q);
    for (int a = 0; a < Q; a++) invfact[a] = gf_inv_host(fact[a]);
    if (upload_vec(c, &c.d_fact, fact) || upload_vec(c, &c.d_invfact, invfact)) return -1;

    std::vector<FieldDesc> vf;
    std::vector<int16_t> rt;
    auto add = [&](int fid, int sel, int width, auto rowfn, int limit = 0, int by_party = 0, int noncanon_bit = -1) {
        FieldDesc fd{};
        fd.noncanon_bit = noncanon_bit;
        fd.off = (uint32_t)P.off[fid];
        fd.sel = sel;
        fd.width = width;
        fd.limit = limit;
        fd.limit_by_party = by_party;
        fd.rowtab_off = (int)rt.size();
        for (int e = 0; e < width; e++) rt.push_back((int16_t)rowfn(e));
        vf.push_back(fd);
    };
    add(F_F, 0, M, [&](int e) { return rm.f + e; });
    add(F_NTTF, 0, M, [&](int e) { return rm.tf + e; });
    add(F_BETA, 1, NCHK, [&](int e) { return rm.beta(e); }, DEG + 1, 1);
    add(F_GAMMA, 1, NCHK, [&](int e) { return rm.gamma(e); }, DEG + 1, 1);
    add(F_S, 0, K, [&](int e) { return rm.s + e; });
    add(F_E, 0, K, [&](int e) { return rm.e + e; });
    add(F_T, 1, K, [&](int e) { return rm.t_in + e; }, DEG + 1);
    add(F_NTTS, 0, K, [&](int e) { return rm.ntts + e; });
    add(F_NTTE, 0, K, [&](int e) { return rm.ntte + e; });
    add(F_NTTAR, 0, K, [&](int e) { return rm.nttar + e; });
    add(F_NTTAS, 0, K, [&](int e) { return rm.nttas + e; });
    add(F_SR, 1, K, [&](int e) { return rm.sr_in + e; }, 0, 0, FB_SR_ER_SHARES);
    add(F_ER, 1, K, [&](int e) { return rm.er_in + e; }, 0, 0, FB_SR_ER_SHARES);
    add(F_SETA, 1, K * E, [&](int e) { return rm.seta_in + e; }, DEG + 1);
    add(F_EETA, 1, K * E, [&](int e) { return rm.eeta_in + e; }, DEG + 1);
    add(F_SSUB, 0, K * E, [&](int e) { return rm.ssub + e; });
    add(F_ESUB, 0, K * E, [&](int e) { return rm.esub + e; });
    add(F_ZS, 0, K * Z, [&](int e) { return rm.zs(e / Z, e % Z); });
    add(F_ZE, 0, K * Z, [&](int e) { return rm.ze(e / Z, e % Z); });
    add(F_US, 1, K * Z, [&](int e) { return rm.us(e / Z, e % Z); }, DEG2 + 1);
    add(F_UE, 1, K * Z, [&](int e) { return rm.ue(e / Z, e % Z); }, DEG2 + 1);
    c.n_vfields = (int)vf.size();
    c.vplan = make_field_plan(vf.data(), c.n_vfields);
    if (upload_vec(c, &c.d_vfields, vf)) return -1;
    if (upload_vec(c, &c.d_vrowtab, rt)) return -1;

    std::vector<int16_t> bg, isrc, idst, urows;
    for (int j = 0; j < NCHK; j++) bg.push_back((int16_t)rm.beta(j));
    for (int j = 0; j < NCHK; j++) bg.push_back((int16_t)rm.gamma(j));
    auto pair = [&](int src0, int dst0, int n) { for (int i = 0; i < n; i++) { isrc.push_back((int16_t)(src0 + i)); idst.push_back((int16_t)(dst0 + i)); } };
    pair(rm.sr_in, rm.sr, K);
    pair(rm.er_in, rm.er, K);
    pair(rm.t_in, rm.t, K);
    pair(rm.seta_in, rm.seta, K * E);
    pair(rm.eeta_in, rm.eeta, K * E);
    for (int i = 0; i < K; i++) for (int k = 0; k < Z; k++) urows.push_back((int16_t)rm.us(i, k));
    for (int i = 0; i < K; i++) for (int k = 0; k < Z; k++) urows.push_back((int16_t)rm.ue(i, k));
    c.n_interp_d = (int)isrc.size();
    c.n_interp_2d = (int)urows.size();
    if (upload_vec(c, &c.d_rows_bg, bg) || upload_vec(c, &c.d_rows_isrc, isrc) || upload_vec(c, &c.d_rows_idst, idst) ||
        upload_vec(c, &c.d_rows_u, urows))
        return -1;

    c.o_stride = (size_t)rm.nrows * OS;
    auto dev = [&](auto **p, size_t per) -> hipError_t {
        const hipError_t e = dalloc(p, B * per);
        if (e == hipSuccess) { c.reg_pp(p, per * sizeof(**p)); c.reg_buf("verifier workspace", p, per * sizeof(**p), Ctx::INV_PER_PROOF, Ctx::INVG_VERIFY); }
        return e;
    };
    HIPCHK(dev(&c.d_O, c.o_stride));
    HIPCHK(hipMemsetAsync(c.d_O, 0, B * c.o_stride * sizeof(uint16_t), c.stream));
    HIPCHK(dev(&c.d_w, (size_t)2 * 832));
    HIPCHK(dev(&c.d_ell, 416));
    HIPCHK(dev(&c.d_node_of, 416));
    HIPCHK(dev(&c.d_isort, (size_t)c.sel_stride));
    HIPCHK(dev(&c.d_hrange, 4));
    HIPCHK(dev(&c.d_gather, interp_y_bytes(0)));
    HIPCHK(dev(&c.d_gather2, interp_y_bytes(1)));
    HIPCHK(dev(&c.d_sec, (size_t)2 * NCHK * 256));
    HIPCHK(dev(&c.d_sec_u1, (size_t)c.n_interp_2d * 256));
    HIPCHK(dev(&c.d_sec_u2, (size_t)c.n_interp_2d * 256));
    HIPCHK(hipHostMalloc(reinterpret_cast<void **>(&c.h_Iimg), B * 2 * NOPEN, hipHostMallocDefault));
    c.reg_pp(&c.h_Iimg, (size_t)2 * NOPEN);
    c.reg_buf("h_Iimg", &c.h_Iimg, (size_t)2 * NOPEN, Ctx::INV_PER_PROOF | Ctx::INV_HOST, Ctx::INVG_VERIFY);
    HIPCHK(dev(&c.d_odig, (size_t)NOPEN * 32));
    HIPCHK(hipHostMalloc(reinterpret_cast<void **>(&c.h_odig), B * NOPEN * 32, hipHostMallocDefault));
    c.reg_pp(&c.h_odig, (size_t)NOPEN * 32);
    c.reg_buf("h_odig", &c.h_odig, (size_t)NOPEN * 32, Ctx::INV_PER_PROOF | Ctx::INV_HOST, Ctx::INVG_VERIFY);
    HIPCHK(hipStreamSynchronize(c.stream));
    c.verify_ready = true;
    return 0;
}

int stage_verifier_inputs(Ctx &c, int n, const uint8_t *pi, const uint8_t *pk, bool registered)
{
    if (n < 1 || n > c.call_cap) { c.err = "batch size out of range"; return -1; }
    HIPCHK(hipSetDevice(c.device));
    const Params &P = c.P;
    parallel_for(c.pool, n, c.nthreads, [&](int b) {
        memcpy(c.h_pk + (size_t)b * c.pk_stride, pk + (size_t)b * P.pk_bytes, P.pk_bytes);
        if (!registered) memcpy(c.h_proof + (size_t)b * c.image_stride, pi + (size_t)b * P.proof_bytes, P.proof_bytes);
    });
    HIPCHK(hipMemcpyAsync(c.d_pk, c.h_pk, (size_t)n * c.pk_stride, hipMemcpyHostToDevice, c.stream));
    c.note_pk_written(n);
    c.path_n[registered ? PATH_COPY_DIRECT : PATH_COPY_STAGED]++;
    if (registered)
        HIPCHK(hipMemcpy2DAsync(c.d_proof, c.image_stride, pi, P.proof_bytes, P.proof_bytes, n, hipMemcpyHostToDevice, c.stream));
    else
        HIPCHK(hipMemcpyAsync(c.d_proof, c.h_proof, (size_t)n * c.image_stride, hipMemcpyHostToDevice, c.stream));
    HIPCHK(launch_decode_pk(c.d_pk, c.pk_stride, c.d_t, c.d_A, c.key_stride, P.K, n, c.stream, c.xof_guard()));
    HIPCHK(stream_sync(c));
    if (device_error_check(c)) return -1;
    return 0;
}

int verify_resident(Ctx &c, int n, uint8_t *ok, int pk_mode, const uint8_t *pk, const VerifySeg *segs)
{
    const uint8_t *himg = c.host_img;
    const size_t himg_stride = c.host_img_stride;
    c.host_img = nullptr;
    if (n < 1 || n > c.call_cap) { c.err = "batch size out of range"; return -1; }
    const VerifySeg whole{n, pk, ok, nullptr, nullptr, nullptr};
    if (!segs) segs = &whole;
    {
        int total = 0;
        for (const VerifySeg *s = segs; s; s = s->next) {
            if (!s->ok) { c.err = "ok output buffer is required"; return -1; }
            if (pk_mode == 1 && !s->pk) { c.err = "pk_mode 1 needs the public keys"; return -1; }
            total += s->count;
        }
        if (total != n) { c.err = "internal: merged call segments do not add up"; return -1; }
    }
    const bool bound = c.bind_n > 0;
    if (bound && segs->next) { c.err = "internal: an armed handle's call in a merged run"; return -1; }
    if (bind_check(c, n)) return -1;
    if (bound && pk_mode == 0 && (c.resident_pk_n < n || c.keys_from_pk_n < n)) {
        c.err = "an armed handle (kosk_set_contexts) cannot verify against instances: there are no public key bytes to bind";
        return -1;
    }
    if (pk_mode == 2 && c.resident_pk_n < n) {
        c.err = "no resident public keys for this batch: pk == NULL needs a key generation (or a verifier staging call) of at least n proofs on this context";
        return -1;
    }
    HIPCHK(hipSetDevice(c.device));
// ... 37 lines not shown
    va.rest = c.d_rest;
    va.sel_stride = c.sel_stride;
    va.fail = c.d_fail;
    va.strict = c.strict_encoding ? 1 : 0;
    oh.proof = c.d_proof;
    oh.image_stride = c.image_stride;
    oh.off_s = (uint32_t)P.off[F_S]; oh.off_e = (uint32_t)P.off[F_E]; oh.off_f = (uint32_t)P.off[F_F];
    oh.off_nttf = (uint32_t)P.off[F_NTTF]; oh.off_zs = (uint32_t)P.off[F_ZS]; oh.off_ze = (uint32_t)P.off[F_ZE];
    oh.P = c.d_P;
    oh.proof_stride = c.proof_stride;
    oh.O = c.d_O;
    oh.o_stride = c.o_stride;
    oh.rm = rm;
    oh.opened = c.d_I;
    oh.sel_stride = c.sel_stride;
    oh.prefix = nullptr;
    oh.out = c.d_dig1;
    const bool split_tables = !c.fs_device && himg != nullptr;
    oh.out_compact = split_tables ? c.d_odig : nullptr;
    const size_t dig_bytes = split_tables ? (size_t)n * NOPEN * 32 : (size_t)n * NPARTY * 32;
    auto table_prep = [&](int r) {
        return std::function<void(int)>([&c, himg, himg_stride, r](int b) {
            const uint8_t *unopened = himg + (size_t)b * himg_stride + c.P.off[r ? F_COMM : F_TCOMM];
            assemble_digest_table(c.h_dig + (size_t)b * NPARTY * 32, c.h_Iimg + (size_t)b * NOPEN, unopened, c.h_odig + (size_t)b * NOPEN * 32);
        });
    };
    if (run_segment(c, Ctx::SEG_V1, n, [&]() -> int {
    HIPCHK(launch_opened_setup(c.d_proof, c.image_stride, P.off[F_I], c.d_I, c.d_rest, c.d_isort, c.d_hrange, c.sel_stride, c.d_fail, n, st));
    if (!c.fs_device) HIPCHK(copy_small(c, c.h_Iimg, 2 * NOPEN, c.d_proof + P.off[F_I], c.image_stride, 2 * NOPEN, n, hipMemcpyDeviceToHost, st));


    const GateOffsets go{(uint32_t)P.off[F_SSUB], (uint32_t)P.off[F_ESUB], (uint32_t)P.off[F_ZS], (uint32_t)P.off[F_ZE]};
    HIPCHK(launch_disassemble(va, c.d_vfields, c.vplan, c.d_vrowtab, c.d_proof, c.image_stride, P.off[F_TCOMM],
                              P.off[F_COMM], c.d_dig1, c.d_dig2, go, n, st));
    c.prof_begin(PR_V_HASH_TCOMM, n);
    HIPCHK(launch_opened_hash(oh, K, false, n, st));
    c.prof_end(PR_V_HASH_TCOMM);
    if (c.fs_device) return 0;
    if (split_tables) HIPCHK(hipMemcpyAsync(c.h_odig, c.d_odig, dig_bytes, hipMemcpyDeviceToHost, st));
    else HIPCHK(copy_round_table(c, c.h_dig, c.d_dig1, n));
    return 0;
    }, c.fs_device ? nullptr : split_tables ? c.h_odig : c.h_dig)) return -1;
    if (issue_bind_values(c, n)) return -1;
    HIPCHK(hipEventRecord(c.ev, st));
    if (c.fs_device) {
        FsArgs fa{};
        fa.in = c.d_dig1; fa.in_stride = (size_t)NPARTY * 32; fa.len = NPARTY * 32;
        fa.alpha = c.d_alpha; fa.alpha_stride = 80; fa.J = P.J;
        fa.bind = bound ? c.d_bind : nullptr;
        c.prof_begin(PR_V_FS_ALPHA, n);
        HIPCHK(launch_fs_chain(fa, FS_ALPHA, n, st));
        c.prof_end(PR_V_FS_ALPHA);
        c.path_n[PATH_FS_DEVICE]++;
    }
    t1 = now_sec(); c.phase_sec[PH_V1_ISSUE] = t1 - t0; t0 = t1;

    if (run_segment(c, Ctx::SEG_V1B, n, [&]() -> int {
    if (pk_mode) HIPCHK(launch_decode_pk(c.d_pk, c.pk_stride, c.d_t, c.d_A, c.key_stride, K, n, st, c.xof_guard()));
    InterpArgs ia{};
    ia.rest = c.d_rest;
    ia.isort = c.d_isort;
    ia.hrange = c.d_hrange;
    ia.sel_stride = c.sel_stride;
    ia.inv = c.d_inv;
    ia.invlimb = c.d_invlimb;
    ia.fact = c.d_fact;
    ia.invfact = c.d_invfact;
    ia.w = c.d_w;
    ia.ell = c.d_ell;
    ia.node_of = c.d_node_of;
    c.prof_begin(PR_V_INTERP_BUILD, n);
    HIPCHK(launch_interp_setup(ia, n, st));
    c.prof_end(PR_V_INTERP_BUILD);
    HIPCHK(launch_gather_frags(c.d_P, c.proof_stride, c.d_rows_isrc, c.n_interp_d, c.d_gather, c.d_rows_u, c.n_interp_2d, c.d_gather2,
                               c.d_rest, c.sel_stride, c.d_w, n, st));
    {
        c.prof_begin(PR_V_GEMM_INTERP, n);
        HIPCHK(launch_interp_apply(ia, c.d_P, c.proof_stride, c.d_rows_isrc, c.d_rows_idst, c.n_interp_d, c.d_gather, c.n_interp_2d,
                                   c.d_gather2, c.d_sec_u1, n, st));
        c.prof_end(PR_V_GEMM_INTERP);
        const GemmSrc gs3{c.d_P, c.proof_stride, c.d_rows_u, RS, NSEC};
        const GemmDst gd3{c.d_sec_u2, (size_t)c.n_interp_2d * 256, nullptr, 256, 0};
        if (gemm_modq(c, c.t_recon_2d, gs3, gd3, c.n_interp_2d, n)) return -1;
        const GemmSrc xs{c.d_P, c.proof_stride, c.d_rows_idst, RS, 0};
        const GemmDst xd{c.d_P, c.proof_stride, c.d_rows_idst, RS, EXP_OFF};
        c.prof_begin(PR_V_GEMM_EXPAND, n);
        if (gemm_modq(c, c.t_expand, xs, xd, c.n_interp_d, n)) return -1;
        c.prof_end(PR_V_GEMM_EXPAND);
    }
    HIPCHK(launch_check_batch(va, c.d_t, c.d_sec_u1, c.d_sec_u2, c.n_interp_2d, n, st));
    NttArgs na{};
    na.in = reinterpret_cast<const int16_t *>(c.d_P);
    na.in_gstride = c.proof_stride;
    na.src_off = c.d_off + c.off_sr_er;
    na.npg = 2 * K;
    na.npoly = 2 * K * n;
    na.out = reinterpret_cast<int16_t *>(c.d_P);
    na.out_gstride = c.proof_stride;
    na.dst_off = c.d_off + c.off_nttsr_er;
    na.out_canonical = 1;
    HIPCHK(launch_relation_ntt(na, c.d_A, c.key_stride, c.d_P, c.proof_stride, rm, n, st));
    {
        const GemmSrc xs{c.d_P, c.proof_stride, c.d_gemm2_rows, RS, 0};
        const GemmDst xd{c.d_P, c.proof_stride, c.d_gemm2_rows, RS, EXP_OFF};
        if (gemm_modq(c, c.t_expand, xs, xd, c.n_gemm2, n)) return -1;
    }
    return 0;
    })) return -1;

    auto any_hook = [&]() {
        bool h = c.round_hook != nullptr;
        for (const VerifySeg *sg = segs; sg; sg = sg->next) h |= sg->hook != nullptr;
        return h;
    };
    const bool hooks = c.fs_device && any_hook();
    if (!c.fs_device || hooks) HIPCHK(wait_event(c, c.ev, 3, n));
    t1 = now_sec(); c.phase_sec[PH_V1_WAIT] = t1 - t0; t0 = t1;
    auto fire_hooks = [&](int rnd, const uint8_t *d_table) {
        bool seg_hooks = false;
        for (const VerifySeg *s = segs; s; s = s->next) seg_hooks |= s->hook != nullptr;
        if (!seg_hooks) {
            if (c.round_hook) c.round_hook(c.round_user, 1, rnd, d_table, (size_t)n * NPARTY * 32);
            return;
        }
        int first = 0;
        for (const VerifySeg *s = segs; s; s = s->next) {
            if (s->hook) s->hook(s->hook_user, 1, rnd, d_table + (size_t)first * NPARTY * 32, (size_t)s->count * NPARTY * 32);
            first += s->count;
        }
    };
    if (!c.fs_device || hooks) fire_hooks(0, c.d_dig1);

    if (!c.fs_device) {
        c.path_n[PATH_FS_HOST]++;
        const std::function<void(int)> prep = table_prep(0);
        fs_alpha_batch(P, n, c.h_dig, (size_t)NPARTY * 32, c.h_alpha, 80, c.nthreads, c.pool, split_tables ? &prep : nullptr, bound ? c.h_bind : nullptr);
    }
    t1 = now_sec(); c.phase_sec[PH_V_FS_ALPHA] = t1 - t0; t0 = t1;
    if (run_segment(c, Ctx::SEG_V2, n, [&]() -> int {
    const uint16_t *alpha_src = c.fs_device ? c.d_alpha : c.h_alpha;

    HIPCHK(launch_pow_table(alpha_src, P.J, P.M, c.d_pwT, n, st));
    LincombArgs la{};
    la.P = c.d_P;
    la.proof_stride = c.proof_stride;
    la.O = c.d_O;
    la.o_stride = c.o_stride;
    la.rm = rm;
    la.J = P.J;
    la.pwT = c.d_pwT;
    la.ncols = NOPEN;
    la.col_map = c.d_I;
    la.col_map_stride = c.sel_stride;
    c.prof_begin(PR_V_LINCOMB, n);
    HIPCHK(launch_lincomb(la, n, st));
    c.prof_end(PR_V_LINCOMB);
    return 0;
    })) return -1;

    oh.prefix = c.d_dig1;
    oh.out = c.d_dig2;
    c.prof_begin(PR_V_HASH_VIEW, n);
    HIPCHK(launch_opened_hash(oh, K, true, n, st));
    c.prof_end(PR_V_HASH_VIEW);
    if (c.fs_device) {
        HIPCHK(hipEventRecord(c.ev, st));
        FsArgs fa{};
        fa.in = c.d_dig2; fa.in_stride = (size_t)NPARTY * 32; fa.len = NPARTY * 32;
        fa.proof = c.d_proof; fa.image_stride = c.image_stride; fa.off_I = (uint32_t)P.off[F_I]; fa.fail = c.d_fail;
        fa.bind = bound ? c.d_bind : nullptr;
        c.prof_begin(PR_V_FS_OPENED, n);
        HIPCHK(launch_fs_chain(fa, FS_CHECK, n, st));
        c.prof_end(PR_V_FS_OPENED);
        c.path_n[PATH_FS_DEVICE]++;
    } else {
        if (split_tables) HIPCHK(hipMemcpyAsync(c.h_odig, c.d_odig, dig_bytes, hipMemcpyDeviceToHost, st));
        else HIPCHK(copy_round_table(c, c.h_dig, c.d_dig2, n));
        HIPCHK(hipEventRecord(c.ev, st));
    }
    t1 = now_sec(); c.phase_sec[PH_V2_ISSUE] = t1 - t0; t0 = t1;

    if (run_segment(c, Ctx::SEG_V2B, n, [&]() -> int {
    NttArgs na{};
    {
        const GemmSrc gs{c.d_P, c.proof_stride, c.d_rows_bg, RS, NSEC};
        const GemmDst gd{c.d_sec, (size_t)2 * NCHK * 256, nullptr, 256, 0};
        c.prof_begin(PR_V_GEMM_RECON, n);
        if (gemm_modq(c, c.t_recon_d, gs, gd, 2 * NCHK, n)) return -1;
// ... 66 lines not shown
```

### mpcith_kyber_kosk_amd/csrc/kosk_verify_kernels.hip

```cpp
#include <hip/hip_runtime.h>

#include <utility>

#include "kosk_device.hpp"
#include "kosk_keccak_dev.hpp"
#include "kosk_keccak_split_dev.hpp"
#include "kosk_math.hpp"

#include <cstdlib>
#include "kosk_cauchy_dev.hpp"
#include "kosk_wave_sync_dev.hpp"

namespace kosk {

constexpr int DIS_TILE = 64 * 80;

__global__ __launch_bounds__(64) void k_disassemble_fields(VerifyArgs v, const FieldDesc *__restrict__ fields, FieldPlan plan,
                                                          const int16_t *__restrict__ rowtab,
                                                          const uint8_t *__restrict__ proof, size_t image_stride, uint32_t off_tcomm,
                                                          uint32_t off_comm, uint8_t *__restrict__ dig1, uint8_t *__restrict__ dig2,
                                                          GateOffsets go)
{
    {
        const int nfb = plan.nrest * NWIN + plan.nopen * ((NOPEN + 63) / 64) + (NREST * 4 + 63) / 64;
// ... 348 lines not shown
    }
    __device__ __forceinline__ v4i frag(int ks, int j, int limb) const { return fb[ks & 1][2 * j + limb]; }
};

template <int SET>
__device__ __forceinline__ void interp_apply_block(const InterpApplyArgs &g, const int b, const int mblk, uint16_t *tab_s, uint16_t *rest_s)
{
    constexpr int KS = SET ? IA_KS2 : IA_KS1, NT = SET ? IA_NT2 : IA_NT1;
    constexpr int NEVAL = SET ? NSEC : DEG + 1;
    const InterpArgs &a = g.ia;
    const int tid = threadIdx.x, lane = tid & 63, wv = tid >> 6;
    const int ncol = SET ? g.n2 : g.n1;
    {
        constexpr int ND = (IA_TAB + 2) / 2, TRIPS = (ND + 255) / 256;
        uint32_t tmp[TRIPS];
#pragma unroll
        for (int i = 0; i < TRIPS; i++) {
            const int idx = tid + i * 256;
            tmp[i] = reinterpret_cast<const uint32_t *>(a.invlimb)[idx < ND ? idx : ND - 1];
        }
#pragma unroll
        for (int i = 0; i < TRIPS; i++) {
            const int idx = tid + i * 256;
            if (idx < ND) reinterpret_cast<uint32_t *>(tab_s)[idx] = tmp[i];
        }
    }
    for (int j = tid; j < KS * 64; j += 256) rest_s[j] = a.rest[(size_t)b * a.sel_stride + j];
    __syncthreads();

    const int m0 = (mblk * 4 + wv) * 16;
    if (m0 >= NEVAL) return;
    const int kq = m0 + (lane & 15) - NSEC + IA_OFF;
    InterpFragsAhead<KS, NT> ld{SET ? g.y2 + (size_t)b * IA_Y2_BYTES : g.y1 + (size_t)b * IA_Y1_BYTES, lane};
    CauchySums<KS, NT> cs;
    cs.template run<IA_TAB>(rest_s, tab_s, lane, kq, ld);
    const int kb = m0 + (lane >> 4) * 4;
    int node[4] = {-1, -1, -1, -1};
    uint32_t ell[4] = {0, 0, 0, 0}, xn[4] = {0, 0, 0, 0};
    if constexpr (!SET) {
#pragma unroll
        for (int r = 0; r < 4; r++)
            if (kb + r <= DEG) { node[r] = a.node_of[(size_t)b * 416 + kb + r]; ell[r] = a.ell[(size_t)b * 416 + kb + r]; }
#pragma unroll
        for (int r = 0; r < 4; r++)
            if (node[r] >= 0) xn[r] = rest_s[node[r]];
    }
#pragma unroll
    for (int j = 0; j < NT; j++) {
        const int col = j * 16 + (lane & 15);
        if (col >= ncol) continue;
        uint32_t v[4];
#pragma unroll
        for (int r = 0; r < 4; r++) v[r] = cs.value(j, r);
        if constexpr (SET) {
            *reinterpret_cast<uint2 *>(g.out2 + ((size_t)b * ncol + col) * NSEC + kb) = make_uint2(v[0] | (v[1] << 16), v[2] | (v[3] << 16));
        } else {
            uint16_t *Pb = g.P + (size_t)b * g.proof_stride;
            const uint16_t *srow = Pb + (size_t)g.src_rows[col] * RS + NSEC;
            uint16_t *drow = Pb + (size_t)g.dst_rows[col] * RS;
#pragma unroll
            for (int r = 0; r < 4; r++)
                if (kb + r <= DEG) drow[kb + r] = node[r] >= 0 ? srow[xn[r]] : (uint16_t)gf_mul(ell[r], v[r]);
        }
    }
}

__global__ __launch_bounds__(256) void k_interp_apply(InterpApplyArgs g, int nproofs)
{
    __shared__ __attribute__((aligned(4))) uint16_t tab_s[IA_TAB + 2];
    __shared__ __attribute__((aligned(16))) uint16_t rest_s[IA_KS2 * 64];
    const int vid = xcd_virtual_id();
    const int b = vid / 11, m = vid % 11;
    if (b >= nproofs) return;
    if (m < 7) interp_apply_block<0>(g, b, m, tab_s, rest_s);
    else interp_apply_block<1>(g, b, m - 7, tab_s, rest_s);
}


__global__ __launch_bounds__(192) void k_check_opened(VerifyArgs v)
{
    const int t = threadIdx.x, b = blockIdx.x, i = blockIdx.y;
    if (t >= NOPEN) return;
    const RowMap &rm = v.rm;
    const uint16_t *Pb = v.P + (size_t)b * v.proof_stride + NSEC + v.opened[(size_t)b * v.sel_stride + t];
    const uint16_t *Ob = v.O + (size_t)b * v.o_stride + t;
    auto at = [&](int row) { return (uint32_t)Pb[(size_t)row * RS]; };
    auto op = [&](int row) { return (uint32_t)Ob[(size_t)row * OS]; };
    constexpr int MAXE = 7;
    const int E = rm.E;
    const uint32_t p_nttsr = at(rm.nttsr + i), p_ntter = at(rm.ntter + i), p_nttasr = at(rm.nttasr + i), p_t = at(rm.t + i);
    const uint32_t o_ntts = op(rm.ntts + i), o_ntte = op(rm.ntte + i), o_nttr_s = op(rm.nttr + i), o_nttr_e = op(rm.nttr + rm.K + i);
    const uint32_t o_nttas = op(rm.nttas + i), o_nttar = op(rm.nttar + i), o_s = op(rm.s + i), o_e = op(rm.e + i);
    uint32_t p_seta[MAXE], p_eeta[MAXE], o_ssub[MAXE], o_esub[MAXE];
#pragma unroll
    for (int m = 0; m < MAXE; m++) {
        const int mm = i * E + min(m, E - 1);
        p_seta[m] = at(rm.seta + mm); p_eeta[m] = at(rm.eeta + mm);
        o_ssub[m] = op(rm.ssub + mm); o_esub[m] = op(rm.esub + mm);
    }
    uint32_t bits = 0;
    if (o_ntts != ref_sub_u16(p_nttsr, o_nttr_s)) bits |= 1u << FB_NTT_S_E;
    if (o_ntte != ref_sub_u16(p_ntter, o_nttr_e)) bits |= 1u << FB_NTT_S_E;
    if (p_nttasr != ref_add_u16(o_nttas, o_nttar)) bits |= 1u << FB_A_SR;
    if (p_t != ref_add_u16(o_nttas, o_ntte)) bits |= 1u << FB_T_RELATION;
#pragma unroll
    for (int m = 0; m < MAXE; m++) {
        if (m < E && o_ssub[m] != ref_sub_u16(o_s, p_seta[m])) bits |= 1u << FB_SUB_ETA;
        if (m < E && o_esub[m] != ref_sub_u16(o_e, p_eeta[m])) bits |= 1u << FB_SUB_ETA;
    }
    if (bits) atomicOr(&v.fail[b], bits);
}



__global__ __launch_bounds__(256) void k_opened_setup(const uint8_t *__restrict__ proof, size_t image_stride, uint32_t off_I,
                                                     uint16_t *__restrict__ I, uint16_t *__restrict__ rest,
                                                     uint16_t *__restrict__ isort, uint16_t *__restrict__ hrange,
                                                     size_t sel_stride, uint32_t *__restrict__ fail)
{
    __shared__ uint32_t cnt[NPARTY];
    __shared__ int bad, wave_used[4], node[3];
    const int t = threadIdx.x, b = blockIdx.x;
    for (int p = t; p < NPARTY; p += 256) cnt[p] = 0;
    if (t == 0) bad = 0;
    __syncthreads();
    uint32_t v = t;
    if (t < NOPEN) {
        v = reinterpret_cast<const uint16_t *>(proof + (size_t)b * image_stride + off_I)[t];
        if (v >= NPARTY || atomicAdd(&cnt[v], 1u) != 0) atomicOr(&bad, 1);
    }
    __syncthreads();
    const bool malformed = bad != 0;
    if (malformed) {
        __syncthreads();
        for (int p = t; p < NPARTY; p += 256) cnt[p] = p < NOPEN;
        v = t;
        __syncthreads();
    }
    if (t < NOPEN) I[(size_t)b * sel_stride + t] = (uint16_t)v;
    int u[6], mine = 0;
#pragma unroll
    for (int k = 0; k < 6; k++) {
        const int p = 6 * t + k;
        u[k] = p < NPARTY && cnt[p] != 0;
        mine += u[k];
    }
    int incl = mine;
#pragma unroll
    for (int d = 1; d < 64; d <<= 1) {
        const int o = __shfl_up(incl, d, 64);
        if ((t & 63) >= d) incl += o;
    }
    if ((t & 63) == 63) wave_used[t >> 6] = incl;
    __syncthreads();
    int used_before = incl - mine;
    for (int w = 0; w < (t >> 6); w++) used_before += wave_used[w];
#pragma unroll
    for (int k = 0; k < 6; k++) {
        const int p = 6 * t + k;
        if (p >= NPARTY) break;
        if ((p & 63) == 0) I[(size_t)b * sel_stride + SEL_WIN + (p >> 6)] = (uint16_t)(p - used_before);
        if (u[k]) {
            isort[(size_t)b * sel_stride + used_before] = (uint16_t)p;
            used_before++;
        } else {
            const int j = p - used_before;
            rest[(size_t)b * sel_stride + j] = (uint16_t)p;
            if (j == 0) node[0] = p;
            if (j == DEG) node[1] = p;
            if (j == DEG2) node[2] = p;
        }
    }
    __syncthreads();
    if (t == 0) {
        uint16_t *hr = hrange + (size_t)b * 4;
        hr[0] = (uint16_t)node[0];
        hr[1] = (uint16_t)(node[1] - DEG);
        hr[2] = (uint16_t)node[0];
        hr[3] = (uint16_t)(node[2] - DEG2);
        fail[b] = malformed ? 1u << FB_MALFORMED : 0u;
        I[(size_t)b * sel_stride + SEL_WIN + NWIN] = (uint16_t)NREST;
    }
}

__global__ __launch_bounds__(256) void k_check_batch(VerifyArgs v, const uint16_t *__restrict__ t_pk,
                                                     const uint16_t *__restrict__ u1, const uint16_t *__restrict__ u2, int nu)
{
    constexpr int NB_REST = (NREST + 255) / 256;
    const int role = blockIdx.x, b = blockIdx.y, t = threadIdx.x;
    const RowMap &rm = v.rm;
    if (role < NB_REST) {
        const int i = role * 256 + t;
        if (i >= NREST) return;
// ... 21 lines not shown
            pt[i] = Pb[(size_t)(rm.t + ii) * RS];
            tk[i] = t_pk[((size_t)b * K + ii) * 256 + t];
        }
#pragma unroll
        for (int i = 0; i < MAXK; i++) bits |= pt[i] != tk[i] ? 1u << FB_T_PK : 0u;
#pragma unroll
        for (int m = 0; m < MAXE; m++) {
            const int mm = min(m, E - 1);
            const uint32_t c = gf_encode(mm - v.eta1);
            uint32_t y[2 * MAXK];
#pragma unroll
            for (int i = 0; i < MAXK; i++) {
                const int ii = min(i, K - 1);
                y[2 * i] = Pb[(size_t)(rm.seta + ii * E + mm) * RS];
                y[2 * i + 1] = Pb[(size_t)(rm.eeta + ii * E + mm) * RS];
            }
#pragma unroll
            for (int i = 0; i < 2 * MAXK; i++) bits |= y[i] != c ? 1u << FB_ETA_CONST : 0u;
        }
        if (bits) atomicOr(&v.fail[b], bits);
    } else {
        const int q = role - NB_REST - 1;
        const uint16_t *x = (q < nu ? u1 : u2) + ((size_t)b * nu + (q < nu ? q : q - nu)) * 256;
        if (x[t] != 0) atomicOr(&v.fail[b], 1u << (q < nu ? FB_U_INTERP : FB_U_RECON));
    }
}

hipError_t launch_check_batch(const VerifyArgs &v, const uint16_t *t_pk, const uint16_t *u1, const uint16_t *u2, int nu, int nproofs,
                              hipStream_t st)
{
    hipLaunchKernelGGL(k_check_batch, dim3((NREST + 255) / 256 + 1 + 2 * nu, nproofs), dim3(256), 0, st, v, t_pk, u1, u2, nu);
    return hipGetLastError();
}
size_t interp_y_bytes(int set) { return set ? IA_Y2_BYTES : IA_Y1_BYTES; }
int interp_table_len() { return IA_TAB + 2; }
int interp_table_off() { return IA_OFF; }
hipError_t launch_gather_frags(const uint16_t *P, size_t proof_stride, const int16_t *rows1, int nrows1, uint8_t *out1,
                               const int16_t *rows2, int nrows2, uint8_t *out2, const uint16_t *rest, int sel_stride,
                               const uint16_t *w, int nproofs, hipStream_t st)
{
    if (nrows1 > 16 * IA_NT1 || nrows2 > 16 * IA_NT2) return hipErrorInvalidValue;
    const int threads = IA_NT1 * 16 * IA_KS1 * 4 + IA_NT2 * 16 * IA_KS2 * 4;
    hipLaunchKernelGGL(k_gather_frags, dim3((threads + 255) / 256, nproofs), dim3(256), 0, st, P, proof_stride, rows1, nrows1, out1, rows2,
                       nrows2, out2, rest, sel_stride, w);
    return hipGetLastError();
}
hipError_t launch_opened_setup(const uint8_t *proof, size_t image_stride, size_t off_I, uint16_t *I, uint16_t *rest, uint16_t *isort,
                               uint16_t *hrange, size_t sel_stride, uint32_t *fail, int nproofs, hipStream_t st)
{
    hipLaunchKernelGGL(k_opened_setup, dim3(nproofs), dim3(256), 0, st, proof, image_stride, (uint32_t)off_I, I, rest, isort, hrange, sel_stride, fail);
    return hipGetLastError();
}
hipError_t launch_disassemble(const VerifyArgs &v, const FieldDesc *fields, const FieldPlan &plan, const int16_t *rowtab,
                              const uint8_t *proof, size_t image_stride, size_t off_tcomm, size_t off_comm,
                              uint8_t *dig1, uint8_t *dig2, const GateOffsets &go, int nproofs, hipStream_t st)
{
    hipLaunchKernelGGL(k_disassemble_fields, dim3(plan.nrest * NWIN + plan.nopen * ((NOPEN + 63) / 64) + (NREST * 4 + 63) / 64 + (NOPEN + 63) / 64, nproofs), dim3(64), 0,
                       st, v, fields, plan, rowtab, proof, image_stride, (uint32_t)off_tcomm, (uint32_t)off_comm, dig1, dig2, go);
    return hipGetLastError();
}
hipError_t launch_interp_setup(const InterpArgs &a, int nproofs, hipStream_t st)
{
    hipLaunchKernelGGL(k_interp_setup, dim3(8 * nproofs), dim3(256), 0, st, a, nproofs);
    return hipGetLastError();
}
hipError_t launch_interp_apply(const InterpArgs &a, uint16_t *P, size_t proof_stride, const int16_t *src_rows, const int16_t *dst_rows,
                               int n1, const uint8_t *y1, int n2, const uint8_t *y2, uint16_t *out2, int nproofs, hipStream_t st)
{
    if (n1 > 16 * IA_NT1 || n2 > 16 * IA_NT2 || n1 < 1 || n2 < 1) return hipErrorInvalidValue;
    InterpApplyArgs g{};
    g.ia = a;
    g.P = P;
    g.proof_stride = proof_stride;
    g.src_rows = src_rows;
    g.dst_rows = dst_rows;
    g.n1 = n1;
    g.y1 = y1;
    g.n2 = n2;
    g.y2 = y2;
    g.out2 = out2;
    hipLaunchKernelGGL(k_interp_apply, dim3((11 * nproofs + 7) / 8 * 8), dim3(256), 0, st, g, nproofs);
    return hipGetLastError();
}
hipError_t launch_check_opened(const VerifyArgs &v, int nproofs, hipStream_t st)
{
    hipLaunchKernelGGL(k_check_opened, dim3(nproofs, v.rm.K), dim3(192), 0, st, v);
    return hipGetLastError();
}

}
```

Baseline: 187,500.

## Evaluate only opened parties in verifier expansion via gathered-point MFMA GEMM

Adds an MFMA int8 GEMM kernel that evaluates the Lagrange expansion only at the opened party points, using a per-party point table. The verifier no longer expands every row to all parties, and the full expansion is narrowed to the sr/er rows. The prover stops storing s-eta/e-eta rows and instead computes them as s minus eta during proof image assembly. This is meant to cut verifier GEMM work and prover stores, at the cost of a new kernel, new tables and extra subtraction logic in assembly.

After: 187,700, median of 2. Within noise of the previous version (+0.1%).

```diff
diff --git a/include/kosk_mi355x.h b/include/kosk_mi355x.h
--- a/include/kosk_mi355x.h
+++ b/include/kosk_mi355x.h
@@ -157,6 +157,8 @@
                            const uint8_t *d_prefix, int with_prefix, uint8_t *d_out);
 int kosk_ntt256_batch(kosk_ctx *ctx, const int16_t *d_in, int16_t *d_out, int n);
 int kosk_lagrange_expand(kosk_ctx *ctx, const uint16_t *d_y407, uint16_t *d_shares, int n);
+int kosk_lagrange_expand_at(kosk_ctx *ctx, const uint16_t *d_y407, int rows_per_group, const uint16_t *d_parties, size_t parties_stride,
+                            int ncols, uint16_t *d_out, int n_groups);
 int kosk_recon_secrets(kosk_ctx *ctx, const uint16_t *d_shares, uint16_t *d_secrets, int n, int two_d);
 int kosk_device_synchronize(kosk_ctx *ctx);
 int kosk_streams(const kosk_ctx *ctx);
diff --git a/mpcith_kyber_kosk_amd/api.py b/mpcith_kyber_kosk_amd/api.py
--- a/mpcith_kyber_kosk_amd/api.py
+++ b/mpcith_kyber_kosk_amd/api.py
@@ -169,6 +169,9 @@
     }
     if not (os.environ.get("KOSK_LIB_PATH") and not hasattr(lib, "kosk_kem_key_set")):
         sig.update(onekey)
+    expand_at = {"kosk_lagrange_expand_at": (C.c_int, [vp, vp, C.c_int, vp, sz, C.c_int, vp, C.c_int])}
+    if not (os.environ.get("KOSK_LIB_PATH") and not hasattr(lib, "kosk_lagrange_expand_at")):
+        sig.update(expand_at)
     for name, (res, args) in sig.items():
         fn = getattr(lib, name)
         fn.restype = res
@@ -201,7 +204,8 @@
            "kosk_kem_keypair_batch", "kosk_kem_check_pk", "kosk_kem_check_sk",
            "kosk_keyseed_value", "kosk_keyseed_device", "kosk_stage_prover_keys_derived", "kosk_prove_keys_derived_batch",
            "kosk_wipe_secrets", "kosk_set_wipe", "kosk_secret_scan", "kosk_wipe_device", "kosk_wipe_timing",
-           "kosk_kem_key_set", "kosk_kem_key_state", "kosk_kem_key_clear", "kosk_kem_enc_key", "kosk_kem_dec_key"]
+           "kosk_kem_key_set", "kosk_kem_key_state", "kosk_kem_key_clear", "kosk_kem_enc_key", "kosk_kem_dec_key",
+           "kosk_lagrange_expand_at"]
 HAS_KEM = hasattr(lib, "kosk_kem_enc_batch")
 
 
@@ -699,7 +703,7 @@
 
     PROFILE_IDS = ["hash_tcomm", "hash_view", "gemm_expand1", "gemm_expand2", "lincomb", "ntt_f", "assemble",
                    "v_hash_tcomm", "v_hash_view", "v_interp_build", "v_gemm_interp", "v_gemm_expand", "v_gemm_recon", "v_lincomb",
-                   "fs_alpha", "fs_opened", "v_fs_alpha", "v_fs_opened"]
+                   "fs_alpha", "fs_opened", "v_fs_alpha", "v_fs_opened", "v_gemm_opened"]
 
     def profile_enable(self, on=True):
         self._chk(lib.kosk_profile_enable(self._h, int(on)), "profile_enable")
@@ -909,6 +913,7 @@
     PATH_KEM_KEY_SETUP = 19
     PATH_KEM_ENC_KEY = 20
     PATH_KEM_DEC_KEY = 21
+    PATH_OPENED_GEMM = 22
 
     def path_count(self, path_id):
         v = C.c_long()
@@ -975,5 +980,8 @@
     def lagrange_expand(self, d_y407, d_shares, n):
         self._chk(lib.kosk_lagrange_expand(self._h, d_y407, d_shares, n), "lagrange_expand")
 
+    def lagrange_expand_at(self, d_y407, rows_per_group, d_parties, parties_stride, ncols, d_out, n_groups):
+        self._chk(lib.kosk_lagrange_expand_at(self._h, d_y407, rows_per_group, d_parties, parties_stride, ncols, d_out, n_groups), "lagrange_expand_at")
+
     def recon_secrets(self, d_shares, d_secrets, n, two_d=False):
         self._chk(lib.kosk_recon_secrets(self._h, d_shares, d_secrets, n, int(two_d)), "recon_secrets")
diff --git a/mpcith_kyber_kosk_amd/csrc/kosk_capi.cpp b/mpcith_kyber_kosk_amd/csrc/kosk_capi.cpp
--- a/mpcith_kyber_kosk_amd/csrc/kosk_capi.cpp
+++ b/mpcith_kyber_kosk_amd/csrc/kosk_capi.cpp
@@ -1829,6 +1829,37 @@
     GUARD_END
 }
 
+int kosk_lagrange_expand_at(kosk_ctx *ctx, const uint16_t *d_y407, int rows_per_group, const uint16_t *d_parties, size_t parties_stride,
+                            int ncols, uint16_t *d_out, int n_groups)
+{
+    if (!ctx) return -1;
+    if (!d_y407 || !d_parties || !d_out || rows_per_group < 1 || n_groups < 1 || ncols < 1 || ncols > OPENED_GEMM_COLS ||
+        parties_stride < (size_t)ncols || parties_stride > 0x7FFFFFFFu)
+        return bad_args(ctx, __func__);
+    GUARD(ctx)
+    Ctx &c = *ctx->c;
+    ctx->clear_err();
+    HIPCHK_C(hipSetDevice(c.device));
+    const int cap = c.own_batch * c.rm.nrows / rows_per_group;
+    if (cap < 1) { c.err = "kosk_lagrange_expand_at: rows_per_group exceeds the handle's row matrix"; return -1; }
+    for (int done = 0; done < n_groups;) {
+        const int m = (n_groups - done) < cap ? (n_groups - done) : cap;
+        HIPCHK_C(launch_rows_copy(d_y407 + (size_t)done * rows_per_group * XLEN, XLEN, c.d_P, RS, XLEN, m * rows_per_group, c.stream));
+        OpenedGemmArgs og{};
+        og.Apt = c.t_expand.dpoint; og.Mtab = NPARTY;
+        og.src = c.d_P; og.src_gstride = (size_t)rows_per_group * RS; og.src_rows = nullptr; og.src_rstride = RS;
+        og.parties = d_parties + (size_t)done * parties_stride; og.parties_stride = (int)parties_stride; og.ncols = ncols;
+        og.out = d_out + (size_t)done * rows_per_group * ncols; og.out_gstride = (size_t)rows_per_group * ncols; og.out_rows = nullptr;
+        og.out_rstride = ncols;
+        og.nrows = rows_per_group; og.ngroups = m;
+        HIPCHK_C(launch_opened_gemm(og, false, c.stream));
+        c.path_n[PATH_OPENED_GEMM]++;
+        done += m;
+    }
+    return 0;
+    GUARD_END
+}
+
 int kosk_recon_secrets(kosk_ctx *ctx, const uint16_t *d_shares, uint16_t *d_secrets, int n, int two_d)
 {
     if (!ctx) return -1;
diff --git a/mpcith_kyber_kosk_amd/csrc/kosk_ctx.cpp b/mpcith_kyber_kosk_amd/csrc/kosk_ctx.cpp
--- a/mpcith_kyber_kosk_amd/csrc/kosk_ctx.cpp
+++ b/mpcith_kyber_kosk_amd/csrc/kosk_ctx.cpp
@@ -1,5 +1,6 @@
 #include "kosk_ctx.hpp"
 
+#include <algorithm>
 #include <atomic>
 
 #include <chrono>
@@ -67,7 +68,7 @@
             if (e) (void)hipEventDestroy(e);
         return;
     }
-    void *dev[] = {t_expand.dfrag, t_recon_d.dfrag, t_recon_2d.dfrag, d_fresh_rows, d_gemm1_rows, d_gemm2_rows, d_off, d_fields, d_asm_groups, d_asm_elems,
+    void *dev[] = {t_expand.dfrag, t_expand.dpoint, d_rows_xfull, d_rows_xopen, t_recon_d.dfrag, t_recon_2d.dfrag, d_fresh_rows, d_gemm1_rows, d_gemm2_rows, d_off, d_fields, d_asm_groups, d_asm_elems,
                    d_rowtab, d_P, d_tape, d_seedbuf, d_dig1, d_dig2, d_proof, d_A, d_se, d_kg, d_sehat, d_t, d_alpha, d_I, d_pwT, d_coef, d_lin_rows,
                    d_gather, d_gather2, d_O, d_w, d_ell, d_sec, d_sec_u1, d_sec_u2, d_fail, d_inv, d_invlimb, d_vfields,
                    d_vrowtab, d_rows_bg, d_rows_isrc, d_rows_idst, d_rows_u, d_fact, d_invfact, d_node_of, d_isort, d_hrange, d_odig, d_bind};
@@ -103,6 +104,18 @@
         }
 }
 
+static void pack_point_table(const std::vector<uint16_t> &A, int M, int Kdim, int KS, std::vector<uint8_t> &out)
+{
+    out.assign((size_t)M * KS * 128, 0);
+    for (int m = 0; m < M; m++)
+        for (int k = 0; k < Kdim; k++) {
+            int c0, c1;
+            limb_split(gf_center(A[(size_t)m * Kdim + k]), c0, c1);
+            out[(size_t)m * KS * 128 + k] = (uint8_t)(int8_t)c0;
+            out[(size_t)m * KS * 128 + KS * 64 + k] = (uint8_t)(int8_t)c1;
+        }
+}
+
 static int upload_table(Ctx &c, GemmTable &t, const std::vector<uint16_t> &A, int M, int Kdim)
 {
     t.M = M;
@@ -275,6 +288,18 @@
             else if (x < NPTS) lagrange_row(&A[(size_t)m * XLEN], XLEN, 0, x);
         }
         if (upload_table(c, c.t_expand, A, EXP_M, XLEN)) return -1;
+        std::vector<uint16_t> Ap((size_t)NPARTY * XLEN, 0);
+        for (int p = 0; p < NPARTY; p++) {
+            const int x = NSEC + p;
+            if (x < EXP_OFF) Ap[(size_t)p * XLEN + x] = 1;
+            else std::copy_n(&A[(size_t)(x - EXP_OFF) * XLEN], XLEN, &Ap[(size_t)p * XLEN]);
+        }
+        std::vector<uint8_t> pk;
+        pack_point_table(Ap, NPARTY, XLEN, c.t_expand.KS, pk);
+        HIPCHK(dalloc(&c.t_expand.dpoint, pk.size()));
+        c.reg_buf("table", &c.t_expand.dpoint, pk.size(), 0);
+        HIPCHK(hipMemcpyAsync(c.t_expand.dpoint, pk.data(), pk.size(), hipMemcpyHostToDevice, c.stream));
+        HIPCHK(hipStreamSynchronize(c.stream));
     }
     {
         std::vector<uint16_t> A((size_t)NSEC * XLEN), A2((size_t)NSEC * (DEG2 + 1));
@@ -348,8 +373,8 @@
     add(F_ER, 1, K, [&](int e) { return rm.er + e; });
     add(F_SETA, 1, K * E, [&](int e) { return rm.seta + e; });
     add(F_EETA, 1, K * E, [&](int e) { return rm.eeta + e; });
-    add(F_SSUB, 0, K * E, [&](int e) { return rm.ssub + e; });
-    add(F_ESUB, 0, K * E, [&](int e) { return rm.esub + e; });
+    add(F_SSUB, 0, K * E, [&](int e) { return rm.seta + e; });
+    add(F_ESUB, 0, K * E, [&](int e) { return rm.eeta + e; });
     add(F_ZS, 0, K * Z, [&](int e) { return rm.zs(e / Z, e % Z); });
     add(F_ZE, 0, K * Z, [&](int e) { return rm.ze(e / Z, e % Z); });
     add(F_US, 1, K * Z, [&](int e) { return rm.us(e / Z, e % Z); });
@@ -368,12 +393,20 @@
             for (int f = 0; f < c.nfields; f++) {
                 const FieldDesc &fd = c.h_fields[f];
                 if (fd.sel != sel) continue;
-                if (g.nsub && (g.nrows + fd.width > 80 || g.nsub == 12)) flush();
+                if (g.nsub && (g.nrows + fd.width > 80 || g.nsub == 12 || fd.off == (uint32_t)P.off[F_S])) flush();
                 if (!g.nsub) { g.sel = sel; g.rowtab_off = (int)c.h_rowtab.size(); g.elem_off = (int)elems.size(); }
                 g.sub_off[g.nsub] = fd.off; g.sub_width[g.nsub] = (int16_t)fd.width; g.sub_col[g.nsub] = (int16_t)g.nrows;
+                const bool is_ssub = fd.off == (uint32_t)P.off[F_SSUB], is_esub = fd.off == (uint32_t)P.off[F_ESUB];
                 for (int k = 0; k < fd.width; k++) {
                     c.h_rowtab.push_back(c.h_rowtab[fd.rowtab_off + k]);
-                    elems.push_back(AsmElem{(int32_t)(fd.off / 2 + k), (int16_t)fd.width, (int16_t)(64 * g.nrows + k)});
+                    int tile = sel ? 64 * g.nrows + k : -1;
+                    if (is_ssub || is_esub) {
+                        const int minuend = (is_ssub ? rm.s : rm.e) + k / E;
+                        for (int r = 0; r < g.nrows; r++)
+                            if (c.h_rowtab[g.rowtab_off + r] == minuend) tile = r;
+                        if (tile < 0) { c.err = "internal: s / e rows are not in the image group of s - eta / e - eta"; return -1; }
+                    }
+                    elems.push_back(AsmElem{(int32_t)(fd.off / 2 + k), (int16_t)fd.width, (int16_t)tile});
                 }
                 g.nrows += fd.width;
                 g.nsub++;
diff --git a/mpcith_kyber_kosk_amd/csrc/kosk_ctx.hpp b/mpcith_kyber_kosk_amd/csrc/kosk_ctx.hpp
--- a/mpcith_kyber_kosk_amd/csrc/kosk_ctx.hpp
+++ b/mpcith_kyber_kosk_amd/csrc/kosk_ctx.hpp
@@ -50,14 +50,15 @@
 
 enum ProfId { PR_HASH_TCOMM = 0, PR_HASH_VIEW, PR_GEMM_EXPAND1, PR_GEMM_EXPAND2, PR_LINCOMB, PR_NTT_F, PR_ASSEMBLE,
               PR_V_HASH_TCOMM, PR_V_HASH_VIEW, PR_V_INTERP_BUILD, PR_V_GEMM_INTERP, PR_V_GEMM_EXPAND, PR_V_GEMM_RECON,
-              PR_V_LINCOMB, PR_FS_ALPHA, PR_FS_OPENED, PR_V_FS_ALPHA, PR_V_FS_OPENED, PR_COUNT };
+              PR_V_LINCOMB, PR_FS_ALPHA, PR_FS_OPENED, PR_V_FS_ALPHA, PR_V_FS_OPENED, PR_V_GEMM_OPENED, PR_COUNT };
 
 enum PathId { PATH_HASH_DMA = 0, PATH_HASH_PLAIN, PATH_TABLE_GEMM, PATH_LIMB_GEMM, PATH_COPY_DIRECT, PATH_COPY_STAGED,
               PATH_GRAPH_REPLAY, PATH_DIGEST_COPY, PATH_SMALL_COPY_KERNEL, PATH_FS_DEVICE, PATH_FS_HOST, PATH_TAPE_EXPAND, PATH_KEM_ENC, PATH_KEM_DEC, PATH_DENSE_FILL, PATH_KEM_KEYPAIR, PATH_KEM_CHECK, PATH_KEYSEED, PATH_WIPE,
-              PATH_KEM_KEY_SETUP, PATH_KEM_ENC_KEY, PATH_KEM_DEC_KEY, PATH_COUNT };
+              PATH_KEM_KEY_SETUP, PATH_KEM_ENC_KEY, PATH_KEM_DEC_KEY, PATH_OPENED_GEMM, PATH_COUNT };
 
 struct GemmTable {
     uint8_t *dfrag = nullptr;
+    uint8_t *dpoint = nullptr;
     int M = 0, Mpad = 0, KS = 0;
 };
 
@@ -211,6 +212,8 @@
     int16_t *d_rows_isrc = nullptr, *d_rows_idst = nullptr;
     int16_t *d_rows_u = nullptr;
     int n_interp_d = 0, n_interp_2d = 0;
+    int16_t *d_rows_xfull = nullptr, *d_rows_xopen = nullptr;
+    int n_xfull = 0, n_xopen = 0;
     uint16_t *d_w = nullptr, *d_ell = nullptr, *d_fact = nullptr, *d_invfact = nullptr;
     int16_t *d_node_of = nullptr;
     uint16_t *d_isort = nullptr, *d_hrange = nullptr;
diff --git a/mpcith_kyber_kosk_amd/csrc/kosk_device.hpp b/mpcith_kyber_kosk_amd/csrc/kosk_device.hpp
--- a/mpcith_kyber_kosk_amd/csrc/kosk_device.hpp
+++ b/mpcith_kyber_kosk_amd/csrc/kosk_device.hpp
@@ -79,6 +79,23 @@
     int ngroups;
 };
 
+constexpr int OPENED_GEMM_COLS = 160;
+struct OpenedGemmArgs {
+    const uint8_t *Apt;
+    int Mtab;
+    const uint16_t *src;
+    size_t src_gstride;
+    const int16_t *src_rows;
+    int src_rstride;
+    const uint16_t *parties;
+    int parties_stride, ncols;
+    uint16_t *out;
+    size_t out_gstride;
+    const int16_t *out_rows;
+    int out_rstride;
+    int nrows, ngroups;
+};
+
 struct LincombArgs {
     uint16_t *P;
     size_t proof_stride;
@@ -315,6 +332,7 @@
                              int nproofs, hipStream_t st);
 bool table_gemm_ok(const GemmArgs &a);
 hipError_t launch_table_gemm(const GemmArgs &a, hipStream_t st);
+hipError_t launch_opened_gemm(const OpenedGemmArgs &a, bool canonical, hipStream_t st);
 hipError_t launch_lincomb_stream(const uint16_t *P, size_t proof_stride, const RowMap &rm, const uint8_t *coef, uint16_t *C,
                                  const int16_t *lin_rows, int J, int nproofs, hipStream_t st);
 hipError_t launch_coef_limbs(const uint16_t *alpha, int J, int M, uint8_t *B, int nproofs, hipStream_t st);
diff --git a/mpcith_kyber_kosk_amd/csrc/kosk_kernels.hip b/mpcith_kyber_kosk_amd/csrc/kosk_kernels.hip
--- a/mpcith_kyber_kosk_amd/csrc/kosk_kernels.hip
+++ b/mpcith_kyber_kosk_amd/csrc/kosk_kernels.hip
@@ -1262,7 +1262,6 @@
             d.v[q] = gf_sub(v.v[q], c[m].v[q]);
             if (m > 0) u.v[q] = gf_sub(gf_mul(m == 1 ? gf_sub(v.v[q], c[0].v[q]) : zd[m > 1 ? m - 2 : 0].v[q], d.v[q]), zd[m > 0 ? m - 1 : 0].v[q]);
         }
-        st8(Pb + (size_t)((who ? rm.esub : rm.ssub) + i * E + m) * RS, d);
         if (m > 0) st8(Pb + (size_t)(who ? rm.ue(i, m - 1) : rm.us(i, m - 1)) * RS, u);
     }
 }
@@ -1395,8 +1394,9 @@
         const AsmElem e0 = el_s[lane], e1 = el_s[lane + 64];
         for (int j = 0; j < nk; j++) {
             const int i = __builtin_amdgcn_readlane(my_pos, j);
-            if (lane < nrows) img16[e0.dst + i * (int)e0.width] = tile[j * nrows + lane];
-            if (NQ > 16 && lane + 64 < nrows) img16[e1.dst + i * (int)e1.width] = tile[j * nrows + lane + 64];
+            const uint16_t *tj = tile + j * nrows;
+            if (lane < nrows) img16[e0.dst + i * (int)e0.width] = e0.tile >= 0 ? (uint16_t)gf_sub(tj[e0.tile], tj[lane]) : tj[lane];
+            if (NQ > 16 && lane + 64 < nrows) img16[e1.dst + i * (int)e1.width] = e1.tile >= 0 ? (uint16_t)gf_sub(tj[e1.tile], tj[lane + 64]) : tj[lane + 64];
         }
     }
 }
diff --git a/mpcith_kyber_kosk_amd/csrc/kosk_verify.cpp b/mpcith_kyber_kosk_amd/csrc/kosk_verify.cpp
--- a/mpcith_kyber_kosk_amd/csrc/kosk_verify.cpp
+++ b/mpcith_kyber_kosk_amd/csrc/kosk_verify.cpp
@@ -110,8 +110,15 @@
     for (int i = 0; i < K; i++) for (int k = 0; k < Z; k++) urows.push_back((int16_t)rm.ue(i, k));
     c.n_interp_d = (int)isrc.size();
     c.n_interp_2d = (int)urows.size();
+    std::vector<int16_t> xfull, xopen;
+    auto run = [](std::vector<int16_t> &v, int row0, int n) { for (int i = 0; i < n; i++) v.push_back((int16_t)(row0 + i)); };
+    run(xfull, rm.sr, K); run(xfull, rm.er, K);
+    run(xopen, rm.t, K); run(xopen, rm.seta, K * E); run(xopen, rm.eeta, K * E);
+    run(xopen, rm.nttsr, K); run(xopen, rm.ntter, K); run(xopen, rm.nttasr, K);
+    c.n_xfull = (int)xfull.size();
+    c.n_xopen = (int)xopen.size();
     if (upload_vec(c, &c.d_rows_bg, bg) || upload_vec(c, &c.d_rows_isrc, isrc) || upload_vec(c, &c.d_rows_idst, idst) ||
-        upload_vec(c, &c.d_rows_u, urows))
+        upload_vec(c, &c.d_rows_u, urows) || upload_vec(c, &c.d_rows_xfull, xfull) || upload_vec(c, &c.d_rows_xopen, xopen))
         return -1;
 
     c.o_stride = (size_t)rm.nrows * OS;
@@ -315,10 +322,10 @@
         const GemmSrc gs3{c.d_P, c.proof_stride, c.d_rows_u, RS, NSEC};
         const GemmDst gd3{c.d_sec_u2, (size_t)c.n_interp_2d * 256, nullptr, 256, 0};
         if (gemm_modq(c, c.t_recon_2d, gs3, gd3, c.n_interp_2d, n)) return -1;
-        const GemmSrc xs{c.d_P, c.proof_stride, c.d_rows_idst, RS, 0};
-        const GemmDst xd{c.d_P, c.proof_stride, c.d_rows_idst, RS, EXP_OFF};
+        const GemmSrc xs{c.d_P, c.proof_stride, c.d_rows_xfull, RS, 0};
+        const GemmDst xd{c.d_P, c.proof_stride, c.d_rows_xfull, RS, EXP_OFF};
         c.prof_begin(PR_V_GEMM_EXPAND, n);
-        if (gemm_modq(c, c.t_expand, xs, xd, c.n_interp_d, n)) return -1;
+        if (gemm_modq(c, c.t_expand, xs, xd, c.n_xfull, n)) return -1;
         c.prof_end(PR_V_GEMM_EXPAND);
     }
     HIPCHK(launch_check_batch(va, c.d_t, c.d_sec_u1, c.d_sec_u2, c.n_interp_2d, n, st));
@@ -334,9 +341,16 @@
     na.out_canonical = 1;
     HIPCHK(launch_relation_ntt(na, c.d_A, c.key_stride, c.d_P, c.proof_stride, rm, n, st));
     {
-        const GemmSrc xs{c.d_P, c.proof_stride, c.d_gemm2_rows, RS, 0};
-        const GemmDst xd{c.d_P, c.proof_stride, c.d_gemm2_rows, RS, EXP_OFF};
-        if (gemm_modq(c, c.t_expand, xs, xd, c.n_gemm2, n)) return -1;
+        OpenedGemmArgs og{};
+        og.Apt = c.t_expand.dpoint; og.Mtab = NPARTY;
+        og.src = c.d_P; og.src_gstride = c.proof_stride; og.src_rows = c.d_rows_xopen; og.src_rstride = RS;
+        og.parties = c.d_I; og.parties_stride = c.sel_stride; og.ncols = NOPEN;
+        og.out = c.d_O; og.out_gstride = c.o_stride; og.out_rows = c.d_rows_xopen; og.out_rstride = OS;
+        og.nrows = c.n_xopen; og.ngroups = n;
+        c.prof_begin(PR_V_GEMM_OPENED, n);
+        HIPCHK(launch_opened_gemm(og, true, st));
+        c.prof_end(PR_V_GEMM_OPENED);
+        if (!c.capturing) c.path_n[PATH_OPENED_GEMM]++;
     }
     return 0;
     })) return -1;
diff --git a/mpcith_kyber_kosk_amd/csrc/kosk_verify_kernels.hip b/mpcith_kyber_kosk_amd/csrc/kosk_verify_kernels.hip
--- a/mpcith_kyber_kosk_amd/csrc/kosk_verify_kernels.hip
+++ b/mpcith_kyber_kosk_amd/csrc/kosk_verify_kernels.hip
@@ -454,20 +454,18 @@
     const int t = threadIdx.x, b = blockIdx.x, i = blockIdx.y;
     if (t >= NOPEN) return;
     const RowMap &rm = v.rm;
-    const uint16_t *Pb = v.P + (size_t)b * v.proof_stride + NSEC + v.opened[(size_t)b * v.sel_stride + t];
     const uint16_t *Ob = v.O + (size_t)b * v.o_stride + t;
-    auto at = [&](int row) { return (uint32_t)Pb[(size_t)row * RS]; };
     auto op = [&](int row) { return (uint32_t)Ob[(size_t)row * OS]; };
     constexpr int MAXE = 7;
     const int E = rm.E;
-    const uint32_t p_nttsr = at(rm.nttsr + i), p_ntter = at(rm.ntter + i), p_nttasr = at(rm.nttasr + i), p_t = at(rm.t + i);
+    const uint32_t p_nttsr = op(rm.nttsr + i), p_ntter = op(rm.ntter + i), p_nttasr = op(rm.nttasr + i), p_t = op(rm.t + i);
     const uint32_t o_ntts = op(rm.ntts + i), o_ntte = op(rm.ntte + i), o_nttr_s = op(rm.nttr + i), o_nttr_e = op(rm.nttr + rm.K + i);
     const uint32_t o_nttas = op(rm.nttas + i), o_nttar = op(rm.nttar + i), o_s = op(rm.s + i), o_e = op(rm.e + i);
     uint32_t p_seta[MAXE], p_eeta[MAXE], o_ssub[MAXE], o_esub[MAXE];
 #pragma unroll
     for (int m = 0; m < MAXE; m++) {
         const int mm = i * E + min(m, E - 1);
-        p_seta[m] = at(rm.seta + mm); p_eeta[m] = at(rm.eeta + mm);
+        p_seta[m] = op(rm.seta + mm); p_eeta[m] = op(rm.eeta + mm);
         o_ssub[m] = op(rm.ssub + mm); o_esub[m] = op(rm.esub + mm);
     }
     uint32_t bits = 0;
@@ -481,6 +479,132 @@
         if (m < E && o_esub[m] != ref_sub_u16(o_e, p_eeta[m])) bits |= 1u << FB_SUB_ETA;
     }
     if (bits) atomicOr(&v.fail[b], bits);
+}
+
+constexpr int OG_NBT = 3, OG_NB = 16 * OG_NBT, OG_KS = 7, OG_WAVES = 4, OG_CHUNKS = OPENED_GEMM_COLS / 16;
+template <bool CANON>
+__global__ __launch_bounds__(64 * OG_WAVES, 2) void k_opened_gemm(OpenedGemmArgs a)
+{
+    constexpr int KS = OG_KS, NBT = OG_NBT, NT = 64 * OG_WAVES;
+    __shared__ __attribute__((aligned(16))) uint8_t ldsB[KS * NBT * 2048];
+    __shared__ __attribute__((aligned(8))) uint16_t p_s[OPENED_GEMM_COLS];
+    const int tid = threadIdx.x, lane = tid & 63, w = tid >> 6;
+    const int bpg = (a.nrows + OG_NB - 1) / OG_NB;
+    const int g = (int)blockIdx.x / bpg, rb = (int)blockIdx.x - g * bpg;
+    if (g >= a.ngroups) return;
+    const uint16_t *srcg = a.src + (size_t)g * a.src_gstride;
+    auto src_row = [&](int i) { return srcg + (size_t)(a.src_rows ? (int)a.src_rows[i] : i) * a.src_rstride; };
+    constexpr int ITEMS = OG_NB * KS * 4, PER = (ITEMS + NT - 1) / NT;
+    uint4 x0[PER], x1[PER];
+#pragma unroll
+    for (int q = 0; q < PER; q++) {
+        const int item = tid + q * NT;
+        const int row_l = item / (KS * 4), kc16 = item - row_l * (KS * 4);
+        x0[q] = make_uint4(0, 0, 0, 0);
+        x1[q] = x0[q];
+        if (item < ITEMS && rb * OG_NB + row_l < a.nrows) {
+            const uint16_t *src = src_row(rb * OG_NB + row_l) + kc16 * 16;
+            x0[q] = *reinterpret_cast<const uint4 *>(src);
+            x1[q] = *reinterpret_cast<const uint4 *>(src + 8);
+        }
+    }
+    for (int i = tid; i < OPENED_GEMM_COLS; i += NT)
+        p_s[i] = (uint16_t)min((int)a.parties[(size_t)g * a.parties_stride + min(i, a.ncols - 1)], a.Mtab - 1);
+#pragma unroll
+    for (int q = 0; q < PER; q++) {
+        const int item = tid + q * NT;
+        if (item < ITEMS) {
+            const int row_l = item / (KS * 4), kc16 = item - row_l * (KS * 4);
+            uint4 lo, hi;
+            if constexpr (CANON) gm_split16_pk(x0[q], x1[q], lo, hi);
+            else gm_split16(x0[q], x1[q], lo, hi);
+            uint8_t *d = ldsB + ((kc16 >> 2) * NBT + (row_l >> 4)) * 2048 + (row_l & 15) * 64 + (((kc16 & 3) ^ limb_swz(row_l & 15)) << 4);
+            *reinterpret_cast<uint4 *>(d) = lo;
+            *reinterpret_cast<uint4 *>(d + 1024) = hi;
+        }
+    }
+    __syncthreads();
+    if (w >= OG_CHUNKS) return;
+    const int frag = (lane & 15) * 64 + (((lane >> 4) ^ limb_swz(lane & 15)) << 4);
+    v4i fa[KS][2];
+    auto load_chunk_ks = [&](int c, int ks, v4i (&dst)[2]) {
+        const int m = p_s[c * 16 + (lane & 15)];
+        const uint8_t *src = a.Apt + (size_t)m * (KS * 128) + ks * 64 + (lane >> 4) * 16;
+        dst[0] = *reinterpret_cast<const v4i *>(src);
+        dst[1] = *reinterpret_cast<const v4i *>(src + KS * 64);
+    };
+#pragma unroll
+    for (int ks = 0; ks < KS; ks++) load_chunk_ks(w, ks, fa[ks]);
+    const uint16_t *irow[NBT];
+    long orow[NBT];
+#pragma unroll
+    for (int j = 0; j < NBT; j++) {
+        const int i = rb * OG_NB + j * 16 + (lane & 15);
+        irow[j] = srcg;
+        orow[j] = -1;
+        if (i < a.nrows) {
+            irow[j] = src_row(i) + NSEC;
+            orow[j] = (long)((size_t)g * a.out_gstride + (size_t)(a.out_rows ? (int)a.out_rows[i] : i) * a.out_rstride);
+        }
+    }
+    const bool wide = a.out_rstride % 4 == 0 && a.out_gstride % 4 == 0 && (reinterpret_cast<uintptr_t>(a.out) & 7) == 0;
+    const v4i zero4 = {0, 0, 0, 0}, bias4 = {LIMB_BIAS, LIMB_BIAS, LIMB_BIAS, LIMB_BIAS};
+    v4i fb[2][2 * NBT], fb0[2 * NBT];
+    auto load_b = [&](int ks, v4i (&dst)[2 * NBT]) {
+        const uint8_t *lb = ldsB + ks * NBT * 2048 + frag;
+#pragma unroll
+        for (int j = 0; j < NBT; j++) {
+            dst[2 * j] = *reinterpret_cast<const v4i *>(lb + j * 2048);
+            dst[2 * j + 1] = *reinterpret_cast<const v4i *>(lb + j * 2048 + 1024);
+        }
+    };
+    load_b(0, fb0);
+    for (int c = w; c < OG_CHUNKS; c += OG_WAVES) {
+        const int cn = c + OG_WAVES < OG_CHUNKS ? c + OG_WAVES : c;
+        const int col = c * 16 + (lane >> 4) * 4;
+        v4i s0[NBT], s1[NBT], s2[NBT];
+#pragma unroll
+        for (int ks = 0; ks < KS; ks++) {
+            v4i(&bc)[2 * NBT] = ks == 0 ? fb0 : fb[ks & 1];
+            v4i(&bn)[2 * NBT] = ks + 1 == KS ? fb0 : fb[(ks & 1) ^ 1];
+            load_b(ks + 1 < KS ? ks + 1 : 0, bn);
+            __builtin_amdgcn_sched_barrier(0);
+#pragma unroll
+            for (int j = 0; j < NBT; j++) s0[j] = __builtin_amdgcn_mfma_i32_16x16x64_i8(fa[ks][0], bc[2 * j], ks == 0 ? bias4 : s0[j], 0, 0, 0);
+#pragma unroll
+            for (int j = 0; j < NBT; j++) s1[j] = __builtin_amdgcn_mfma_i32_16x16x64_i8(fa[ks][0], bc[2 * j + 1], ks == 0 ? zero4 : s1[j], 0, 0, 0);
+#pragma unroll
+            for (int j = 0; j < NBT; j++) s1[j] = __builtin_amdgcn_mfma_i32_16x16x64_i8(fa[ks][1], bc[2 * j], s1[j], 0, 0, 0);
+#pragma unroll
+            for (int j = 0; j < NBT; j++) s2[j] = __builtin_amdgcn_mfma_i32_16x16x64_i8(fa[ks][1], bc[2 * j + 1], ks == 0 ? zero4 : s2[j], 0, 0, 0);
+            load_chunk_ks(cn, ks, fa[ks]);
+            __builtin_amdgcn_sched_barrier(0);
+        }
+#pragma unroll
+        for (int j = 0; j < NBT; j++) {
+            uint32_t v[4];
+#pragma unroll
+            for (int r = 0; r < 4; r++) v[r] = gf_reduce_limbs_biased_lazy(s0[j][r], s1[j][r], s2[j][r]);
+            const uint32_t c01 = gf_canon_pair(v[0], v[1]), c23 = gf_canon_pair(v[2], v[3]);
+            v[0] = c01 & 0xFFFFu; v[1] = c01 >> 16; v[2] = c23 & 0xFFFFu; v[3] = c23 >> 16;
+            if (orow[j] < 0) continue;
+            if constexpr (!CANON) {
+#pragma unroll
+                for (int r = 0; r < 4; r++) {
+                    const uint32_t party = p_s[col + r];
+                    if (party < (uint32_t)(EXP_OFF - NSEC)) v[r] = irow[j][party];
+                }
+            }
+            uint16_t *dst = a.out + orow[j] + col;
+            if (wide && col + 4 <= a.ncols) {
+                *reinterpret_cast<uint2 *>(dst) = make_uint2(v[0] | (v[1] << 16), v[2] | (v[3] << 16));
+            } else {
+#pragma unroll
+                for (int r = 0; r < 4; r++)
+                    if (col + r < a.ncols) dst[r] = (uint16_t)v[r];
+            }
+        }
+    }
 }
 
 
@@ -668,6 +792,17 @@
     hipLaunchKernelGGL(k_interp_apply, dim3((11 * nproofs + 7) / 8 * 8), dim3(256), 0, st, g, nproofs);
     return hipGetLastError();
 }
+hipError_t launch_opened_gemm(const OpenedGemmArgs &a, bool canonical, hipStream_t st)
+{
+    if (a.nrows <= 0 || a.ngroups <= 0) return hipSuccess;
+    if (!a.Apt || a.Mtab < 1 || !a.src || !a.parties || !a.out || a.ncols < 1 || a.ncols > OPENED_GEMM_COLS || a.src_rstride % 8 != 0 ||
+        a.src_gstride % 8 != 0 || (reinterpret_cast<uintptr_t>(a.src) & 15) != 0)
+        return hipErrorInvalidValue;
+    const dim3 grid((unsigned)((a.nrows + OG_NB - 1) / OG_NB * a.ngroups));
+    if (canonical) hipLaunchKernelGGL(k_opened_gemm<true>, grid, dim3(64 * OG_WAVES), 0, st, a);
+    else hipLaunchKernelGGL(k_opened_gemm<false>, grid, dim3(64 * OG_WAVES), 0, st, a);
+    return hipGetLastError();
+}
 hipError_t launch_check_opened(const VerifyArgs &v, int nproofs, hipStream_t st)
 {
     hipLaunchKernelGGL(k_check_opened, dim3(nproofs, v.rm.K), dim3(192), 0, st, v);
```
